# Frojdholm/rayrs

Measured on AMD Instinct MI355X. Metric: Mray/s (primary+secondary) on 1M-tri scene @1024spp, higher is better.
Workload: dtype f64

## Files before the change

### include/rayrs_hip.h

```cpp
#ifndef RAYRS_HIP_H
#define RAYRS_HIP_H

#include <stdint.h>

#ifdef __cplusplus
extern "C" {
#endif

typedef enum {
    RAYRS_OK = 0,
    RAYRS_INVALID_ARG = -1,
    RAYRS_HIP_ERROR = -2,
    RAYRS_OOM = -3,
    RAYRS_NO_DEVICE = -4,
    RAYRS_UNSUPPORTED = -5,
    RAYRS_IO_ERROR = -6,
    RAYRS_RCCL_ERROR = -7
} rayrs_status;

const char* rayrs_strerror(int status);
const char* rayrs_last_error(void);


enum {
// ... 3 lines not shown
    RAYRS_MAT_GLASS = 3,
    RAYRS_MAT_COOK_TORRANCE = 4,
    RAYRS_MAT_COOK_TORRANCE_REFRACT = 5,
    RAYRS_MAT_COOK_TORRANCE_GLASS = 6,
    RAYRS_MAT_PLASTIC = 7,
    RAYRS_MAT_NO_REFLECT = 8
};

typedef struct {
    int32_t kind;
    int32_t metallic;
    double color[3];
    double spec_color[3];
    double alpha;
    double ior;
    double r0[3];
} rayrs_material;

typedef struct {
    int32_t emissive;
    int32_t pad;
    double strength;
    double color[3];
} rayrs_emission;

enum { RAYRS_AXIS_X = 0, RAYRS_AXIS_XREV = 1, RAYRS_AXIS_Y = 2, RAYRS_AXIS_YREV = 3, RAYRS_AXIS_Z = 4, RAYRS_AXIS_ZREV = 5 };

enum { RAYRS_BVH_MIDPOINT = 0, RAYRS_BVH_SAH = 1 };


typedef struct rayrs_objects rayrs_objects;

int rayrs_objects_create(rayrs_objects** out);
void rayrs_objects_destroy(rayrs_objects* objs);
uint64_t rayrs_objects_len(const rayrs_objects* objs);

int rayrs_object_sphere(rayrs_objects* objs, double radius, const double origin[3], const rayrs_material* mat,
                        const rayrs_emission* emission);
int rayrs_object_plane(rayrs_objects* objs, int axis, double umin, double umax, double vmin, double vmax, double pos,
                       const rayrs_material* mat, const rayrs_emission* emission);
int rayrs_object_triangle(rayrs_objects* objs, const double p1[3], const double p2[3], const double p3[3],
                          const rayrs_material* mat, const rayrs_emission* emission);
int rayrs_object_from_triangles_f32(rayrs_objects* objs, const float* verts, uint32_t nverts, const uint32_t* idx,
                                    uint32_t ntris, const rayrs_material* mat, const rayrs_emission* emission);
int rayrs_object_from_triangles_f64(rayrs_objects* objs, const double* verts, uint32_t nverts, const uint32_t* idx,
                                    uint32_t ntris, const rayrs_material* mat, const rayrs_emission* emission);
int rayrs_object_from_spheres(rayrs_objects* objs, double radius, const double* centers, uint32_t n,
                              const rayrs_material* mat, const rayrs_emission* emission);
int rayrs_object_box_geom(rayrs_objects* objs, const double lower_left[3], const double upper_right[3],
                          const rayrs_material* mat, const rayrs_emission* emission);


typedef struct rayrs_scene rayrs_scene;

int rayrs_scene_new(const rayrs_objects* objs, double z_near, double z_far, int heuristic, uint32_t splits,
                    uint32_t hdri_w, uint32_t hdri_h, const float* hdri_rgb, int device, rayrs_scene** out);
void rayrs_scene_destroy(rayrs_scene* scene);

typedef struct {
    uint64_t n_objects;
    uint32_t n_interior;
    uint32_t n_prims;
    uint32_t root_ref;
    uint32_t depth;
    uint32_t compact;
    uint32_t n_surfaces;
    uint32_t node_bytes;
    uint32_t prim_bytes;
    uint64_t device_bytes;
    double root_box[6];
    double build_seconds;
    uint32_t n_wide;
    uint32_t wide_root_ref;
    uint32_t wide_depth;
    uint32_t local_pool;
    uint32_t gate_n_wide;
    uint32_t gate_root_ref;
    uint32_t gate_depth;
    uint32_t hot_n_wide;
    uint32_t hot_root_ref;
    uint32_t hot_depth;
    uint32_t hot_first;
    uint32_t hot_count;
    uint32_t hot_pad;
    double hot_box[6];
} rayrs_scene_info_t;

int rayrs_scene_info(const rayrs_scene* scene, rayrs_scene_info_t* info);
int rayrs_scene_clone_to_device(const rayrs_scene* scene, int device, rayrs_scene** out);
int rayrs_scene_device(const rayrs_scene* scene);
int rayrs_scene_export_bvh(const rayrs_scene* scene, double* child_box, uint32_t* child_ref, uint32_t* prim_object);
int rayrs_scene_export_wide(const rayrs_scene* scene, double* wide_box, uint32_t* wide_ref);
int rayrs_scene_export_gate_tree(const rayrs_scene* scene, double* wide_box, uint32_t* wide_ref);
int rayrs_scene_export_hot_tree(const rayrs_scene* scene, double* wide_box, uint32_t* wide_ref);


typedef struct {
    double origin[3];
    double e_x[3];
    double e_y[3];
    double z[3];
    double width, height;
    uint32_t ppc;
    uint32_t x_pixels;
    uint32_t y_pixels;
} rayrs_camera;

int rayrs_camera_new(const double origin[3], const double up[3], const double lookat[3], double fov, double width,
                     double height, uint32_t ppi, rayrs_camera* out);


enum { RAYRS_OUT_F32 = 0, RAYRS_OUT_F64 = 1 };

typedef struct {
    uint32_t spp;
    uint32_t max_bounces;
    uint64_t seed;
    uint32_t sample_chunk;
    uint32_t tile_rank, tile_ranks;
    uint32_t out_format;
    uint32_t count_work;
    uint32_t fast_traversal;
} rayrs_render_params;

typedef struct {
    uint64_t rays;
    uint64_t paths;
    uint64_t nan_pixels;
    uint64_t neg_pixels;
    uint64_t interior_visits;
    uint64_t tri_tests;
    uint64_t sphere_tests;
    uint64_t plane_tests;
    uint64_t escaped_paths;
    uint64_t step_wave, step_lane, inner_wave, leaf_wave;
    uint64_t interior_ticks, leaf_ticks;
    double kernel_ms;
    double total_ms;
    uint64_t kernel_launches;
    double trace_ms;
    uint64_t refill_ticks;
    uint64_t surface_hits[8];
    uint64_t direct_rays;
    double hit_ms, miss_ms;
    uint32_t local_pool;
    uint32_t exact_walk;
    uint32_t hot_group;
    uint32_t stats_pad;
    uint64_t pre_rays;
    uint64_t pre_root_records;
    uint64_t hot_lane;
    uint64_t hot_prim_tests;
    uint64_t hot_tri_divided;
} rayrs_render_stats;

uint32_t rayrs_frame_sample_chunk(uint32_t x_pixels, uint32_t y_pixels, uint32_t spp, uint32_t requested);

int rayrs_render(rayrs_scene* scene, const rayrs_camera* camera, const rayrs_render_params* params, void* out_host,
                 rayrs_render_stats* stats);

int rayrs_render_launch(rayrs_scene* scene, const rayrs_camera* camera, const rayrs_render_params* params,
                        void* out_device, void* hip_stream);
int rayrs_render_finish(rayrs_scene* scene, rayrs_render_stats* stats);

int rayrs_render_multi(rayrs_scene* const* scenes, uint32_t n, const rayrs_camera* camera,
                       const rayrs_render_params* params, void* out_host, rayrs_render_stats* stats);

typedef struct {
    uint32_t pool_slots;
    uint32_t local_pool;
} rayrs_tuning;
int rayrs_scene_set_tuning(rayrs_scene* scene, const rayrs_tuning* tuning);

typedef struct rayrs_film rayrs_film;

typedef struct {
    uint32_t sample_chunk;
    uint32_t max_bounces;
    uint64_t seed;
    uint32_t tile_rank, tile_ranks;
    uint32_t fast_traversal;
    uint32_t pad;
} rayrs_film_params;

typedef struct {
    uint64_t samples;
    uint64_t full_chunks;
    uint64_t rays, paths;
    uint64_t nan_pixels, neg_pixels;
    uint64_t unconverged, nonfinite;
    uint32_t closed;
    uint32_t pad;
} rayrs_film_status;

int rayrs_film_create(rayrs_scene* scene, const rayrs_camera* camera, const rayrs_film_params* params, rayrs_film** out);
void rayrs_film_destroy(rayrs_film* film);
int rayrs_film_render(rayrs_film* film, uint32_t n, rayrs_render_stats* pass_stats);
int rayrs_film_render_adaptive(rayrs_film* film, uint32_t n, double tau, uint32_t max_tile_samples,
                               uint64_t* active_tiles, rayrs_render_stats* pass_stats);
uint64_t rayrs_film_tile_samples(rayrs_film* film, uint32_t* out, uint64_t cap);
int rayrs_film_read(rayrs_film* film, uint32_t out_format, void* out_host);
int rayrs_film_status_get(rayrs_film* film, double tau, rayrs_film_status* out);
uint64_t rayrs_film_state_bytes(const rayrs_film* film);
int rayrs_film_state_get(rayrs_film* film, void* out_host, uint64_t cap);
int rayrs_film_state_set(rayrs_film* film, const void* in_host, uint64_t bytes);


int rayrs_render_features(rayrs_scene* scene, const rayrs_camera* camera, uint32_t samples, uint64_t seed, uint32_t tile_rank,
                          uint32_t tile_ranks, uint32_t fast_traversal, double* normal, double* albedo, double* depth,
                          double* coverage, uint32_t* object);
int rayrs_film_features(rayrs_film* film, uint32_t samples, double* normal, double* albedo, double* depth, double* coverage,
                        uint32_t* object);
int rayrs_film_denoise(rayrs_film* film, uint32_t feature_samples, uint32_t levels, double kn, double ka, double kz, double kc,
                       uint32_t out_format, void* out_host);
int rayrs_image_denoise(int device, uint32_t w, uint32_t h, const double* color, const double* normal, const double* albedo,
                        const double* depth, uint32_t levels, double kn, double ka, double kz, double kc, double* out);

#define RAYRS_ABI_VERSION 7
uint32_t rayrs_abi_version(void);

uint32_t rayrs_abi_layout(uint32_t* out, uint32_t cap);


const char* rayrs_io_last_error(void);
void rayrs_buffer_free(void* p);

int rayrs_ply_load(const char* path, float** verts, uint32_t* nverts, uint32_t** idx, uint32_t* ntris);
int rayrs_ply_save(const char* path, const float* verts, uint32_t nverts, const uint32_t* idx, uint32_t ntris,
                   int binary);
int rayrs_obj_load(const char* path, double** verts, uint32_t* nverts, uint32_t** idx, uint32_t* ntris);
int rayrs_obj_load_spheres(const char* path, double** centers, uint32_t* n);
// ... 11 lines not shown
```

### rayrs_amd/_ffi.py

```python
import ctypes as C
import os

_HERE = os.path.dirname(os.path.abspath(__file__))
LIB_PATH = os.environ.get("RAYRS_HIP_LIB") or os.path.join(_HERE, "librayrs_hip.so")

SYMBOLS = [
    "rayrs_strerror", "rayrs_last_error",
    "rayrs_objects_create", "rayrs_objects_destroy", "rayrs_objects_len",
    "rayrs_object_sphere", "rayrs_object_plane", "rayrs_object_triangle",
    "rayrs_object_from_triangles_f32", "rayrs_object_from_triangles_f64",
    "rayrs_object_from_spheres", "rayrs_object_box_geom",
    "rayrs_scene_new", "rayrs_scene_destroy", "rayrs_scene_info", "rayrs_scene_export_bvh",
    "rayrs_scene_export_wide", "rayrs_scene_export_gate_tree", "rayrs_scene_export_hot_tree", "rayrs_scene_clone_to_device", "rayrs_scene_device", "rayrs_scene_set_tuning",
    "rayrs_camera_new",
    "rayrs_frame_sample_chunk", "rayrs_render", "rayrs_render_launch", "rayrs_render_finish", "rayrs_render_multi",
    "rayrs_film_create", "rayrs_film_destroy", "rayrs_film_render", "rayrs_film_read", "rayrs_film_status_get",
    "rayrs_film_state_bytes", "rayrs_film_state_get", "rayrs_film_state_set",
    "rayrs_film_render_adaptive", "rayrs_film_tile_samples",
    "rayrs_render_features", "rayrs_film_features", "rayrs_film_denoise", "rayrs_image_denoise",
    "rayrs_abi_layout", "rayrs_abi_version",
    "rayrs_io_last_error", "rayrs_buffer_free", "rayrs_ply_load", "rayrs_ply_save", "rayrs_obj_load", "rayrs_obj_load_spheres",
    "rayrs_hdr_load", "rayrs_hdr_save", "rayrs_image_to_bytes", "rayrs_ppm_save", "rayrs_png_save",
]


PRIVATE_SYMBOLS = ["rayrs_test_math", "rayrs_test_rng", "rayrs_test_intersect", "rayrs_test_trace", "rayrs_test_path_trace", "rayrs_test_material", "rayrs_test_background",
                   "rayrs_lab_set", "rayrs_lab_round_ms", "rayrs_lab_multi_rehearse"]


class MaterialDesc(C.Structure):
    _fields_ = [("kind", C.c_int32), ("metallic", C.c_int32), ("color", C.c_double * 3),
                ("spec_color", C.c_double * 3), ("alpha", C.c_double), ("ior", C.c_double),
                ("r0", C.c_double * 3)]


class EmissionDesc(C.Structure):
    _fields_ = [("emissive", C.c_int32), ("pad", C.c_int32), ("strength", C.c_double),
                ("color", C.c_double * 3)]


class CameraDesc(C.Structure):
    _fields_ = [("origin", C.c_double * 3), ("e_x", C.c_double * 3), ("e_y", C.c_double * 3),
                ("z", C.c_double * 3), ("width", C.c_double), ("height", C.c_double),
                ("ppc", C.c_uint32), ("x_pixels", C.c_uint32), ("y_pixels", C.c_uint32)]


class SceneInfo(C.Structure):
    _fields_ = [("n_objects", C.c_uint64), ("n_interior", C.c_uint32), ("n_prims", C.c_uint32),
                ("root_ref", C.c_uint32), ("depth", C.c_uint32), ("compact", C.c_uint32),
                ("n_surfaces", C.c_uint32), ("node_bytes", C.c_uint32), ("prim_bytes", C.c_uint32),
                ("device_bytes", C.c_uint64), ("root_box", C.c_double * 6),
                ("build_seconds", C.c_double), ("n_wide", C.c_uint32), ("wide_root_ref", C.c_uint32),
                ("wide_depth", C.c_uint32), ("local_pool", C.c_uint32), ("gate_n_wide", C.c_uint32),
                ("gate_root_ref", C.c_uint32), ("gate_depth", C.c_uint32),
                ("hot_n_wide", C.c_uint32), ("hot_root_ref", C.c_uint32), ("hot_depth", C.c_uint32),
                ("hot_first", C.c_uint32), ("hot_count", C.c_uint32), ("hot_pad", C.c_uint32),
                ("hot_box", C.c_double * 6)]


class RenderParams(C.Structure):
    _fields_ = [("spp", C.c_uint32), ("max_bounces", C.c_uint32), ("seed", C.c_uint64),
                ("sample_chunk", C.c_uint32), ("tile_rank", C.c_uint32), ("tile_ranks", C.c_uint32),
                ("out_format", C.c_uint32), ("count_work", C.c_uint32), ("fast_traversal", C.c_uint32)]


class RenderStats(C.Structure):
    _fields_ = [("rays", C.c_uint64), ("paths", C.c_uint64), ("nan_pixels", C.c_uint64),
                ("neg_pixels", C.c_uint64), ("interior_visits", C.c_uint64), ("tri_tests", C.c_uint64),
                ("sphere_tests", C.c_uint64), ("plane_tests", C.c_uint64), ("escaped_paths", C.c_uint64),
                ("step_wave", C.c_uint64), ("step_lane", C.c_uint64), ("inner_wave", C.c_uint64),
                ("leaf_wave", C.c_uint64), ("interior_ticks", C.c_uint64), ("leaf_ticks", C.c_uint64),
                ("kernel_ms", C.c_double), ("total_ms", C.c_double), ("kernel_launches", C.c_uint64),
                ("trace_ms", C.c_double), ("refill_ticks", C.c_uint64),
                ("surface_hits", C.c_uint64 * 8), ("direct_rays", C.c_uint64), ("hit_ms", C.c_double), ("miss_ms", C.c_double),
                ("local_pool", C.c_uint32), ("exact_walk", C.c_uint32), ("hot_group", C.c_uint32),
                ("stats_pad", C.c_uint32), ("pre_rays", C.c_uint64), ("pre_root_records", C.c_uint64), ("hot_lane", C.c_uint64),
                ("hot_prim_tests", C.c_uint64), ("hot_tri_divided", C.c_uint64)]

    def as_dict(self):
        d = {n: getattr(self, n) for n, _ in self._fields_}
        d["surface_hits"] = list(self.surface_hits)
        return d


class Tuning(C.Structure):
    _fields_ = [("pool_slots", C.c_uint32), ("local_pool", C.c_uint32)]


class FilmParams(C.Structure):
    _fields_ = [("sample_chunk", C.c_uint32), ("max_bounces", C.c_uint32), ("seed", C.c_uint64),
                ("tile_rank", C.c_uint32), ("tile_ranks", C.c_uint32), ("fast_traversal", C.c_uint32), ("pad", C.c_uint32)]


class FilmStatus(C.Structure):
    _fields_ = [("samples", C.c_uint64), ("full_chunks", C.c_uint64), ("rays", C.c_uint64), ("paths", C.c_uint64),
                ("nan_pixels", C.c_uint64), ("neg_pixels", C.c_uint64), ("unconverged", C.c_uint64),
                ("nonfinite", C.c_uint64), ("closed", C.c_uint32), ("pad", C.c_uint32)]

    def as_dict(self):
        return {n: getattr(self, n) for n, _ in self._fields_ if n != "pad"}


class LabTuning(C.Structure):
    _fields_ = [("refill_min", C.c_uint32), ("leaf_min", C.c_uint32), ("static_pct", C.c_uint32),
                ("stack_lds", C.c_uint32), ("hot_records", C.c_uint32), ("trav_blocks_per_cu", C.c_uint32),
                ("eager_light", C.c_uint32), ("local_reserve", C.c_uint32), ("local_segment_items", C.c_uint32),
                ("force_rccl", C.c_uint32), ("gate_tree", C.c_uint32), ("hot_group", C.c_uint32), ("leaf_wait", C.c_uint32), ("flat_blocks_per_cu", C.c_uint32)]


ABI_VERSION = 7

ABI_STRUCTS = [MaterialDesc, EmissionDesc, CameraDesc, SceneInfo, RenderParams, RenderStats, Tuning, FilmParams, FilmStatus]

_lib = None


def lib():
    global _lib
    if _lib is not None:
        return _lib
    if not os.path.exists(LIB_PATH):
        raise RuntimeError(
            f"{LIB_PATH} is missing: build it with `python -c 'import __graft_entry__ as g; g.build()'` "
            "(make -C rayrs_amd/csrc). There is no CPU fallback.")
    L = C.CDLL(LIB_PATH)
    L.rayrs_abi_version.argtypes = []
    L.rayrs_abi_version.restype = C.c_uint32
    if L.rayrs_abi_version() != ABI_VERSION:
        raise RuntimeError(f"{LIB_PATH} has RAYRS_ABI_VERSION {L.rayrs_abi_version()}, this binding was written against "
                           f"{ABI_VERSION}: rebuild the library (make -C rayrs_amd/csrc)")
    dp = C.POINTER(C.c_double)
    vp = C.c_void_p
    L.rayrs_strerror.restype = C.c_char_p
    L.rayrs_strerror.argtypes = [C.c_int]
    L.rayrs_last_error.restype = C.c_char_p
    L.rayrs_objects_create.argtypes = [C.POINTER(vp)]
    L.rayrs_objects_destroy.argtypes = [vp]
    L.rayrs_objects_destroy.restype = None
    L.rayrs_objects_len.argtypes = [vp]
    L.rayrs_objects_len.restype = C.c_uint64
    mp, ep = C.POINTER(MaterialDesc), C.POINTER(EmissionDesc)
    L.rayrs_object_sphere.argtypes = [vp, C.c_double, dp, mp, ep]
    L.rayrs_object_plane.argtypes = [vp, C.c_int] + [C.c_double] * 5 + [mp, ep]
    L.rayrs_object_triangle.argtypes = [vp, dp, dp, dp, mp, ep]
    L.rayrs_object_from_triangles_f32.argtypes = [vp, vp, C.c_uint32, vp, C.c_uint32, mp, ep]
    L.rayrs_object_from_triangles_f64.argtypes = [vp, vp, C.c_uint32, vp, C.c_uint32, mp, ep]
    L.rayrs_object_from_spheres.argtypes = [vp, C.c_double, vp, C.c_uint32, mp, ep]
    L.rayrs_object_box_geom.argtypes = [vp, dp, dp, mp, ep]
    L.rayrs_scene_new.argtypes = [vp, C.c_double, C.c_double, C.c_int, C.c_uint32, C.c_uint32, C.c_uint32, vp,
                                  C.c_int, C.POINTER(vp)]
    L.rayrs_scene_destroy.argtypes = [vp]
    L.rayrs_scene_destroy.restype = None
    L.rayrs_scene_info.argtypes = [vp, C.POINTER(SceneInfo)]
    L.rayrs_scene_export_bvh.argtypes = [vp, vp, vp, vp]
    L.rayrs_scene_export_wide.argtypes = [vp, vp, vp]
    L.rayrs_scene_export_gate_tree.argtypes = [vp, vp, vp]
    L.rayrs_scene_export_hot_tree.argtypes = [vp, vp, vp]
    L.rayrs_scene_clone_to_device.argtypes = [vp, C.c_int, C.POINTER(vp)]
    L.rayrs_scene_device.argtypes = [vp]
# ... 82 lines not shown
```

### rayrs_amd/csrc/abi.cpp

```cpp
#include <hip/hip_runtime.h>

#include <cmath>
#include <cstddef>
#include <cstdlib>
#include <cstring>
#include <memory>
#include <new>
#include <stdexcept>
#include <string>
#include <vector>

#include "../../include/rayrs_hip.h"
#include "film.h"
#include "kernels.h"
#include "local_pool.h"
#include "rayrs_lab.h"
#include "scene_host.hpp"
#include "scene_internal.hpp"
#include "wavefront.h"

using namespace rayrs;

namespace {
thread_local std::string g_last_error;
// ... 217 lines not shown
    for (const SurfaceDev& sf : s->surfaces) ls.kind_mask |= 1u << (uint32_t)sf.kind;
    s->local_ok = true;
}

extern "C++" int rayrs::scene_upload(rayrs_scene* s) {
    HIP_TRY(hipSetDevice(s->device));
    hipDeviceProp_t prop;
    HIP_TRY(hipGetDeviceProperties(&prop, s->device));
    s->cu_count = prop.multiProcessorCount;
    const FlatScene& f = s->flat;
    for (int x = 0; x < 3; x++) {
        const WalkTree& t = s->tree(x);
        if (x == 2 && !f.has_hot) continue;
        HIP_TRY(s->trav[x].d_nodes.upload(t.node_bytes.data(), t.node_bytes.size()));
    }
    if (f.has_hot) HIP_TRY(s->d_hot.upload(&f.hot, sizeof(HotGroupDev)));
    HIP_TRY(s->d_prims.upload(f.prim_bytes.data(), f.prim_bytes.size()));
    HIP_TRY(s->d_surfaces.upload(s->surfaces.data(), s->surfaces.size() * sizeof(SurfaceDev)));
    HIP_TRY(s->d_hdri.upload(f.hdri_quads.data(), f.hdri_quads.size() * sizeof(float)));
    HIP_TRY(s->d_counters.reserve(sizeof(Counters)));
    for (auto& e : s->ev) HIP_TRY(e.create());
    s->device_bytes = f.walk.node_bytes.size() + f.gate.node_bytes.size() + (f.has_hot ? f.gate_hot.node_bytes.size() : 0) + f.prim_bytes.size() + s->surfaces.size() * sizeof(SurfaceDev) +
                      f.hdri_quads.size() * sizeof(float);
    RAYRS_TRY(scene_configure_traversal(s));
    HIP_TRY(s->pool.d_ctl.reserve(sizeof(WfCtl)));
    HIP_TRY(s->pool.h_live.alloc(2 * sizeof(uint32_t)));
    for (auto& e : s->pool.ev_batch) HIP_TRY(e.create());
    HIP_TRY(s->d_next_item.reserve(sizeof(unsigned long long)));
    if (s->local_ok) {
        HIP_TRY(lp_configure());
        HIP_TRY(lp_occupancy(s->flat.compact, s->local.n_prims, (uint32_t)s->surfaces.size(), &s->local_blocks_per_cu));
        if (s->local_blocks_per_cu < 1) s->local_blocks_per_cu = 1;
        if (s->local_blocks_per_cu > (int)LP_WPS) s->local_blocks_per_cu = (int)LP_WPS;
        HIP_TRY(s->d_local_items.reserve(LOCAL_MAX_SEGMENTS * sizeof(unsigned long long)));
    }
    return RAYRS_OK;
}

int rayrs_scene_new(const rayrs_objects* objs, double z_near, double z_far, int heuristic, uint32_t splits,
                    uint32_t hdri_w, uint32_t hdri_h, const float* hdri_rgb, int device, rayrs_scene** out) {
    RAYRS_GUARDED({
    if (!objs || !out) return RAYRS_INVALID_ARG;
    *out = nullptr;
    std::unique_ptr<rayrs_scene> s(new rayrs_scene());
    RAYRS_TRY(build_flat_scene(objs->list, z_near, z_far, heuristic, splits, hdri_w, hdri_h, hdri_rgb, &s->flat));
    if (std::max(s->flat.walk.depth, s->flat.gate.depth) > 4096u) {
        g_last_error = "walk tree needs " + std::to_string(std::max(s->flat.walk.depth, s->flat.gate.depth)) + " stack entries (limit 4096)";
        return RAYRS_UNSUPPORTED;
    }
    s->surfaces = objs->list.surfaces;
    s->n_objects = objs->list.objs.size();
    s->device = device;
    scene_configure_local(s.get());
    if (device >= 0) RAYRS_TRY(scene_upload(s.get()));
    *out = s.release();
    return RAYRS_OK;
    })
}

int rayrs_scene_info(const rayrs_scene* scene, rayrs_scene_info_t* info) {
    if (!scene || !info) return RAYRS_INVALID_ARG;
    const FlatScene& f = scene->flat;
    std::memset(info, 0, sizeof(*info));
    info->n_objects = scene->n_objects;
    info->n_interior = f.n_interior();
    info->n_prims = f.n_prims();
    info->root_ref = f.root_ref;
    info->depth = f.depth;
    info->compact = f.compact ? 1u : 0u;
    info->n_surfaces = (uint32_t)scene->surfaces.size();
    info->node_bytes = f.compact ? (uint32_t)sizeof(Node4F32) : (uint32_t)sizeof(Node4F64);
    info->n_wide = f.walk.n();
    info->wide_root_ref = f.walk.root_ref;
    info->wide_depth = f.walk.depth;
    info->gate_n_wide = f.gate.n();
    info->gate_root_ref = f.gate.root_ref;
    info->gate_depth = f.gate.depth;
    if (f.has_hot) {
        info->hot_n_wide = f.gate_hot.n();
        info->hot_root_ref = f.gate_hot.root_ref;
        info->hot_depth = f.gate_hot.depth;
        info->hot_first = f.hot.first;
        info->hot_count = f.hot.count;
        for (int i = 0; i < 6; i++) info->hot_box[i] = f.hot.box[i];
    }
    info->local_pool = (scene->local_ok && scene->tuning.local_pool != 1u) ? 1u : 0u;
    info->prim_bytes = 4u * (f.compact ? PRIM_DWORDS_COMPACT : PRIM_DWORDS_FULL);
    info->device_bytes = scene->device_bytes;
    for (int i = 0; i < 6; i++) info->root_box[i] = f.root_box[i];
    info->build_seconds = f.build_seconds;
    return RAYRS_OK;
}

int rayrs_scene_export_bvh(const rayrs_scene* scene, double* child_box, uint32_t* child_ref, uint32_t* prim_object) {
    if (!scene) return RAYRS_INVALID_ARG;
    const FlatScene& f = scene->flat;
    if (child_box && !f.child_box.empty()) std::memcpy(child_box, f.child_box.data(), f.child_box.size() * 8);
    if (child_ref && !f.child_ref.empty()) std::memcpy(child_ref, f.child_ref.data(), f.child_ref.size() * 4);
    if (prim_object && !f.prim_object.empty())
        std::memcpy(prim_object, f.prim_object.data(), f.prim_object.size() * 4);
    return RAYRS_OK;
}

static int export_tree(const WalkTree& t, double* wide_box, uint32_t* wide_ref) {
    if (wide_box && !t.box.empty()) std::memcpy(wide_box, t.box.data(), t.box.size() * 8);
    if (wide_ref && !t.ref.empty()) std::memcpy(wide_ref, t.ref.data(), t.ref.size() * 4);
    return RAYRS_OK;
}

int rayrs_scene_export_wide(const rayrs_scene* scene, double* wide_box, uint32_t* wide_ref) {
    return scene ? export_tree(scene->flat.walk, wide_box, wide_ref) : RAYRS_INVALID_ARG;
}

int rayrs_scene_export_gate_tree(const rayrs_scene* scene, double* wide_box, uint32_t* wide_ref) {
    return scene ? export_tree(scene->flat.gate, wide_box, wide_ref) : RAYRS_INVALID_ARG;
}

int rayrs_scene_export_hot_tree(const rayrs_scene* scene, double* wide_box, uint32_t* wide_ref) {
    return scene && scene->flat.has_hot ? export_tree(scene->flat.gate_hot, wide_box, wide_ref) : RAYRS_INVALID_ARG;
}

int rayrs_scene_clone_to_device(const rayrs_scene* scene, int device, rayrs_scene** out) {
    RAYRS_GUARDED({
        if (!scene || !out || device < 0) return RAYRS_INVALID_ARG;
        *out = nullptr;
        std::unique_ptr<rayrs_scene> s(new rayrs_scene());
        s->flat = scene->flat;
        s->surfaces = scene->surfaces;
        s->n_objects = scene->n_objects;
        s->tuning = scene->tuning;
        s->lab = scene->lab;
        s->device = device;
        scene_configure_local(s.get());
        RAYRS_TRY(scene_upload(s.get()));
        *out = s.release();
        return RAYRS_OK;
    })
}

int rayrs_scene_device(const rayrs_scene* scene) { return scene ? scene->device : -1; }

static int scene_quiesce(rayrs_scene* scene) {
    if (scene->device >= 0) {
        HIP_TRY(hipSetDevice(scene->device));
        if (scene->pending && scene->last_stream) {
            HIP_TRY(hipStreamSynchronize(scene->last_stream));
            scene->pending = false;
        }
    }
    return RAYRS_OK;
}

rayrs_scene::~rayrs_scene() {
    if (device < 0) return;
    (void)hipSetDevice(device);
    if (pending && last_stream) (void)hipStreamSynchronize(last_stream);
}

int rayrs_scene_set_tuning(rayrs_scene* scene, const rayrs_tuning* tuning) {
    if (!scene || !tuning) return RAYRS_INVALID_ARG;
    if (tuning->local_pool > 1u) return RAYRS_INVALID_ARG;
    RAYRS_TRY(scene_quiesce(scene));
    scene->tuning = *tuning;
    return RAYRS_OK;
}

// ... 8 lines not shown
}
#endif

static int round_event(rayrs_scene::Pool& pl, uint32_t r, uint32_t k, hipStream_t stream) {
    while (pl.ev_round.size() < 4 * (size_t)(r + 1)) {
        Event e;
        HIP_TRY(e.create());
        pl.ev_round.push_back(std::move(e));
    }
    HIP_TRY(hipEventRecord(pl.ev_round[4 * (size_t)r + k], stream));
    return RAYRS_OK;
}

static int round_ms(const rayrs_scene* scene, uint32_t r, float ms[3]) {
    const Event* e = &scene->pool.ev_round[4 * (size_t)r];
    ms[1] = ms[2] = 0.f;
    HIP_TRY(hipEventElapsedTime(&ms[0], e[0], e[1]));
    if (scene->last_local) return RAYRS_OK;
    HIP_TRY(hipEventElapsedTime(&ms[1], e[1], e[2]));
    HIP_TRY(hipEventElapsedTime(&ms[2], e[2], e[3]));
    return RAYRS_OK;
}

extern "C" int rayrs_lab_round_ms(rayrs_scene* scene, float* out, uint32_t cap_rounds) {
    if (!scene || scene->device < 0 || scene->pending) return RAYRS_INVALID_ARG;
    HIP_TRY(hipSetDevice(scene->device));
    for (uint32_t r = 0; r < scene->pool.timed_rounds && r < cap_rounds && out; r++) RAYRS_TRY(round_ms(scene, r, out + 3 * r));
    return (int)scene->pool.timed_rounds;
}

int rayrs_lab_set(rayrs_scene* scene, const rayrs_lab_tuning* lab) {
    if (!scene || !lab) return RAYRS_INVALID_ARG;
    if (lab->stack_lds > 64u) return RAYRS_INVALID_ARG;
    if (lab->hot_group != 0u && lab->hot_group != 0xffffffffu) return RAYRS_INVALID_ARG;
    if (lab->static_pct > 100u || lab->refill_min > 64u || lab->leaf_min > 64u || lab->leaf_wait > 64u || lab->flat_blocks_per_cu > 64u || lab->eager_light > 1u || lab->force_rccl > 1u || lab->gate_tree > 1u)
        return RAYRS_INVALID_ARG;
    if (lab->local_reserve != 0u && (lab->local_reserve < 8u || lab->local_reserve > 4096u)) return RAYRS_INVALID_ARG;
    if (lab->local_segment_items != 0u && lab->local_segment_items < 65536u) return RAYRS_INVALID_ARG;
    RAYRS_TRY(scene_quiesce(scene));
    scene->lab = *lab;
    if (scene->device >= 0) return scene_configure_traversal(scene);
    return RAYRS_OK;
}

uint32_t rayrs_frame_sample_chunk(uint32_t x_pixels, uint32_t y_pixels, uint32_t spp, uint32_t requested) {
    if (spp == 0) return 0;
    uint64_t chunk = requested ? requested : 4u;
    const uint64_t pixels = (uint64_t)((x_pixels + 7u) / 8u) * ((y_pixels + 7u) / 8u) * 64u;
    while (chunk < spp && pixels * ((spp + chunk - 1) / chunk) > (1ull << 30)) chunk *= 2;
    return chunk >= spp ? 0u : (uint32_t)chunk;
}

uint32_t rayrs_abi_version(void) { return RAYRS_ABI_VERSION; }

uint32_t rayrs_abi_layout(uint32_t* out, uint32_t cap) {
    std::vector<uint32_t> t;
    t.push_back(RAYRS_ABI_VERSION);
#define RAYRS_STRUCT(T, N) t.push_back((uint32_t)sizeof(T)), t.push_back(N)
#define RAYRS_FIELD(T, F) t.push_back((uint32_t)offsetof(T, F))
    RAYRS_STRUCT(rayrs_material, 7);
    RAYRS_FIELD(rayrs_material, kind), RAYRS_FIELD(rayrs_material, metallic), RAYRS_FIELD(rayrs_material, color);
    RAYRS_FIELD(rayrs_material, spec_color), RAYRS_FIELD(rayrs_material, alpha), RAYRS_FIELD(rayrs_material, ior);
    RAYRS_FIELD(rayrs_material, r0);
    RAYRS_STRUCT(rayrs_emission, 4);
    RAYRS_FIELD(rayrs_emission, emissive), RAYRS_FIELD(rayrs_emission, pad), RAYRS_FIELD(rayrs_emission, strength);
    RAYRS_FIELD(rayrs_emission, color);
    RAYRS_STRUCT(rayrs_camera, 9);
    RAYRS_FIELD(rayrs_camera, origin), RAYRS_FIELD(rayrs_camera, e_x), RAYRS_FIELD(rayrs_camera, e_y);
    RAYRS_FIELD(rayrs_camera, z), RAYRS_FIELD(rayrs_camera, width), RAYRS_FIELD(rayrs_camera, height);
    RAYRS_FIELD(rayrs_camera, ppc), RAYRS_FIELD(rayrs_camera, x_pixels), RAYRS_FIELD(rayrs_camera, y_pixels);
    RAYRS_STRUCT(rayrs_scene_info_t, 26);
    RAYRS_FIELD(rayrs_scene_info_t, n_objects), RAYRS_FIELD(rayrs_scene_info_t, n_interior);
    RAYRS_FIELD(rayrs_scene_info_t, n_prims), RAYRS_FIELD(rayrs_scene_info_t, root_ref);
    RAYRS_FIELD(rayrs_scene_info_t, depth), RAYRS_FIELD(rayrs_scene_info_t, compact);
    RAYRS_FIELD(rayrs_scene_info_t, n_surfaces), RAYRS_FIELD(rayrs_scene_info_t, node_bytes);
    RAYRS_FIELD(rayrs_scene_info_t, prim_bytes), RAYRS_FIELD(rayrs_scene_info_t, device_bytes);
    RAYRS_FIELD(rayrs_scene_info_t, root_box), RAYRS_FIELD(rayrs_scene_info_t, build_seconds);
    RAYRS_FIELD(rayrs_scene_info_t, n_wide), RAYRS_FIELD(rayrs_scene_info_t, wide_root_ref);
    RAYRS_FIELD(rayrs_scene_info_t, wide_depth), RAYRS_FIELD(rayrs_scene_info_t, local_pool);
    RAYRS_FIELD(rayrs_scene_info_t, gate_n_wide), RAYRS_FIELD(rayrs_scene_info_t, gate_root_ref);
    RAYRS_FIELD(rayrs_scene_info_t, gate_depth);
    RAYRS_FIELD(rayrs_scene_info_t, hot_n_wide), RAYRS_FIELD(rayrs_scene_info_t, hot_root_ref);
    RAYRS_FIELD(rayrs_scene_info_t, hot_depth), RAYRS_FIELD(rayrs_scene_info_t, hot_first);
    RAYRS_FIELD(rayrs_scene_info_t, hot_count), RAYRS_FIELD(rayrs_scene_info_t, hot_pad);
    RAYRS_FIELD(rayrs_scene_info_t, hot_box);
    RAYRS_STRUCT(rayrs_render_params, 9);
    RAYRS_FIELD(rayrs_render_params, spp), RAYRS_FIELD(rayrs_render_params, max_bounces);
    RAYRS_FIELD(rayrs_render_params, seed), RAYRS_FIELD(rayrs_render_params, sample_chunk);
    RAYRS_FIELD(rayrs_render_params, tile_rank), RAYRS_FIELD(rayrs_render_params, tile_ranks);
    RAYRS_FIELD(rayrs_render_params, out_format), RAYRS_FIELD(rayrs_render_params, count_work);
    RAYRS_FIELD(rayrs_render_params, fast_traversal);
    RAYRS_STRUCT(rayrs_render_stats, 33);
    RAYRS_FIELD(rayrs_render_stats, rays), RAYRS_FIELD(rayrs_render_stats, paths);
    RAYRS_FIELD(rayrs_render_stats, nan_pixels), RAYRS_FIELD(rayrs_render_stats, neg_pixels);
    RAYRS_FIELD(rayrs_render_stats, interior_visits), RAYRS_FIELD(rayrs_render_stats, tri_tests);
    RAYRS_FIELD(rayrs_render_stats, sphere_tests), RAYRS_FIELD(rayrs_render_stats, plane_tests);
    RAYRS_FIELD(rayrs_render_stats, escaped_paths), RAYRS_FIELD(rayrs_render_stats, step_wave);
    RAYRS_FIELD(rayrs_render_stats, step_lane), RAYRS_FIELD(rayrs_render_stats, inner_wave);
    RAYRS_FIELD(rayrs_render_stats, leaf_wave), RAYRS_FIELD(rayrs_render_stats, interior_ticks);
    RAYRS_FIELD(rayrs_render_stats, leaf_ticks), RAYRS_FIELD(rayrs_render_stats, kernel_ms);
    RAYRS_FIELD(rayrs_render_stats, total_ms), RAYRS_FIELD(rayrs_render_stats, kernel_launches);
    RAYRS_FIELD(rayrs_render_stats, trace_ms), RAYRS_FIELD(rayrs_render_stats, refill_ticks);
    RAYRS_FIELD(rayrs_render_stats, surface_hits), RAYRS_FIELD(rayrs_render_stats, direct_rays);
    RAYRS_FIELD(rayrs_render_stats, hit_ms), RAYRS_FIELD(rayrs_render_stats, miss_ms);
    RAYRS_FIELD(rayrs_render_stats, local_pool), RAYRS_FIELD(rayrs_render_stats, exact_walk);
    RAYRS_FIELD(rayrs_render_stats, hot_group), RAYRS_FIELD(rayrs_render_stats, stats_pad);
    RAYRS_FIELD(rayrs_render_stats, pre_rays), RAYRS_FIELD(rayrs_render_stats, pre_root_records);
    RAYRS_FIELD(rayrs_render_stats, hot_lane);
    RAYRS_FIELD(rayrs_render_stats, hot_prim_tests), RAYRS_FIELD(rayrs_render_stats, hot_tri_divided);
    RAYRS_STRUCT(rayrs_tuning, 2);
    RAYRS_FIELD(rayrs_tuning, pool_slots), RAYRS_FIELD(rayrs_tuning, local_pool);
    RAYRS_STRUCT(rayrs_film_params, 7);
    RAYRS_FIELD(rayrs_film_params, sample_chunk), RAYRS_FIELD(rayrs_film_params, max_bounces);
    RAYRS_FIELD(rayrs_film_params, seed), RAYRS_FIELD(rayrs_film_params, tile_rank);
    RAYRS_FIELD(rayrs_film_params, tile_ranks), RAYRS_FIELD(rayrs_film_params, fast_traversal);
    RAYRS_FIELD(rayrs_film_params, pad);
    RAYRS_STRUCT(rayrs_film_status, 10);
    RAYRS_FIELD(rayrs_film_status, samples), RAYRS_FIELD(rayrs_film_status, full_chunks);
    RAYRS_FIELD(rayrs_film_status, rays), RAYRS_FIELD(rayrs_film_status, paths);
    RAYRS_FIELD(rayrs_film_status, nan_pixels), RAYRS_FIELD(rayrs_film_status, neg_pixels);
    RAYRS_FIELD(rayrs_film_status, unconverged), RAYRS_FIELD(rayrs_film_status, nonfinite);
    RAYRS_FIELD(rayrs_film_status, closed), RAYRS_FIELD(rayrs_film_status, pad);
#undef RAYRS_STRUCT
#undef RAYRS_FIELD
    for (uint32_t i = 0; i < cap && i < t.size(); i++) out[i] = t[i];
    return (uint32_t)t.size();
}


int rayrs_camera_new(const double origin[3], const double up[3], const double lookat[3], double fov, double width,
                     double height, uint32_t ppi, rayrs_camera* out) {
    return camera_new(origin, up, lookat, fov, width, height, ppi, out);
}


extern "C++" SceneDev rayrs::make_scene_dev(const rayrs_scene* s, bool exact) {
    SceneDev sc;
    std::memset(&sc, 0, sizeof(sc));
    const int which = s->walk_index(exact);
    const WalkTree& t = s->tree(which);
    const rayrs_scene::Walk& w = s->trav[which];
    sc.hot = which == 2 ? s->d_hot.as<HotGroupDev>() : nullptr;
    sc.nodes = w.d_nodes.as<>();
    sc.prims = s->d_prims.as<>();
    sc.surfaces = s->d_surfaces.as<SurfaceDev>();
    sc.hdri = s->d_hdri.as<float>();
    sc.hdri_w = s->flat.hdri_w;
    sc.hdri_h = s->flat.hdri_h;
    sc.hdri_wm1 = (double)(s->flat.hdri_w - 1u);
    sc.hdri_hm1 = (double)(s->flat.hdri_h - 1u);
    sc.root_ref = t.root_ref;
    sc.stack_depth = t.depth ? t.depth : 1;
    sc.stack_lds = w.stack_lds;
    sc.hot_records = w.hot_records;
    sc.leafq = w.leafq;
    sc.n_surfaces = (uint32_t)s->surfaces.size();
    for (int i = 0; i < 6; i++) sc.root_box[i] = s->flat.root_box[i];
    sc.t0 = s->flat.t0;
    sc.t1 = s->flat.t1;
    sc.exact = exact ? 1u : 0u;
    return sc;
}

constexpr double RAYRS_FAR_DIAGONALS = 8.0;
constexpr double RAYRS_FAR_PRIMITIVES = 4096.0;
extern "C++" bool rayrs::camera_is_far(const rayrs_scene* s, const rayrs_camera* c) {
    const double* b = s->flat.root_box;
    double d2 = 0.0, e2 = 0.0;
    for (int a = 0; a < 3; a++) {
        const double lo = b[2 * a], hi = b[2 * a + 1], o = c->origin[a];
        const double out = o < lo ? lo - o : (o > hi ? o - hi : 0.0);
        d2 += out * out;
        e2 += (hi - lo) * (hi - lo);
    }
    const double small = s->flat.small_extent;
    return d2 > RAYRS_FAR_DIAGONALS * RAYRS_FAR_DIAGONALS * e2 || (small > 0.0 && d2 > RAYRS_FAR_PRIMITIVES * RAYRS_FAR_PRIMITIVES * small * small);
}

extern "C++" CameraDev rayrs::make_camera_dev(const rayrs_camera* c) {
    CameraDev cam;
    std::memset(&cam, 0, sizeof(cam));
    for (int i = 0; i < 3; i++) {
        cam.origin[i] = c->origin[i];
        cam.e_x[i] = c->e_x[i];
        cam.e_y[i] = c->e_y[i];
        cam.z[i] = c->z[i];
    }
    cam.width = c->width;
    cam.height = c->height;
    cam.ppc = (double)c->ppc;
    cam.W = c->x_pixels;
    cam.H = c->y_pixels;
    return cam;
}

extern "C++" uint32_t rayrs::trav_settings(const rayrs_scene* s, bool exact, uint32_t np, RenderDev& rp) {
    const rayrs_lab_tuning& lab = s->lab;
    rp.refill_min = lab.refill_min ? lab.refill_min : 52u;
    rp.leaf_min = lab.leaf_min ? lab.leaf_min : (exact ? 48u : lab.gate_tree ? 32u : 24u);
    rp.leaf_wait = lab.leaf_wait ? lab.leaf_wait : 16u;
    uint32_t trav_bpc = (uint32_t)s->trav[s->walk_index(exact)].blocks_per_cu;
    if (lab.trav_blocks_per_cu && lab.trav_blocks_per_cu < trav_bpc) trav_bpc = lab.trav_blocks_per_cu;
    const uint32_t blocks = (uint32_t)s->cu_count * trav_bpc;
    const uint32_t static_pct = lab.static_pct ? lab.static_pct : 50u;
    const uint64_t n_waves = (uint64_t)blocks * 4u;
    rp.static_windows = (uint32_t)((uint64_t)(np / wf_window_slots()) * static_pct / 100u / n_waves * n_waves);
    return blocks;
}

extern "C++" WfDev rayrs::pool_wf(const DevBuf& block, uint32_t np, const DevBuf& ctl, uint32_t trav_blocks, const DevBuf& spill) {
    WfDev wf;
    std::memset(&wf, 0, sizeof(wf));
    wf.slots = block.as<PathSlot>();
    wf.light = reinterpret_cast<double*>(wf.slots + np);
    wf.state = reinterpret_cast<uint8_t*>(wf.light + (size_t)np * 4u);
    wf.ctl = ctl.as<WfCtl>();
    wf.np = np;
    wf.trav_threads = trav_blocks * 256u;
    wf.stack_spill = spill.as<uint32_t>();
    return wf;
}

struct FramePlan {
    SceneDev sc;
    CameraDev cam;
    RenderDev rp;
    bool exact, eager_light, use_local;
    uint64_t partial_need;
    uint64_t tile_items, seg_tiles, seg_items;
    uint32_t local_blocks;
    uint64_t live_total;
    uint32_t np, trav_blocks, flat_blocks;
    size_t spill_words;
    bool is_film;
    FilmPassDev film;
};

static RenderDev make_render_dev(const rayrs_scene* scene, const rayrs_camera* camera, const rayrs_render_params* params, uint32_t sample0,
                                 const FilmPassDev* film, void* out_device) {
    RenderDev rp;
    std::memset(&rp, 0, sizeof(rp));
    rp.spp = params->spp;
    rp.sample0 = sample0;
// ... 90 lines not shown
        lp.item_count = rp.total_items - lp.item_base < p.seg_items ? rp.total_items - lp.item_base : p.seg_items;
        RenderDev rseg = rp;
        rseg.partial_item0 = lp.item_base;
        const uint64_t share = lp.item_count / ((uint64_t)p.local_blocks * 4u * 16u);
        lp.reserve = (uint32_t)(share < 8u ? 8u : share > 256u ? 256u : share);
        if (scene->lab.local_reserve) lp.reserve = scene->lab.local_reserve;
        lp.pad = 0;
        RAYRS_TRY(round_event(pl, (uint32_t)seg, 0, stream));
        HIP_TRY(lp_launch(scene->flat.compact, rp.count_work != 0u, p.sc, scene->local, p.cam, rseg, lp, p.local_blocks, stream));
        RAYRS_TRY(round_event(pl, (uint32_t)seg, 1, stream));
        const uint32_t seg_lt0 = (uint32_t)(seg * p.seg_tiles), seg_n_lt = (uint32_t)(lp.item_count / p.tile_items);
        HIP_TRY(p.is_film ? launch_film_accumulate(p.cam, rseg, p.film, seg_lt0, seg_n_lt, stream) : launch_resolve(p.cam, rseg, seg_lt0, seg_n_lt, stream));
        pl.timed_rounds = (uint32_t)seg + 1;
    }
    scene->rounds = (uint32_t)n_seg;
    return RAYRS_OK;
}

static int enqueue_streaming(rayrs_scene* scene, const FramePlan& p, const WfDev& wf, hipStream_t stream) {
    rayrs_scene::Pool& pl = scene->pool;
    const RenderDev& rp = p.rp;
    uint32_t* h_live = pl.h_live.as<uint32_t>();
    HIP_TRY(wf_launch_init(wf, (uint32_t)p.live_total, stream));
    HIP_TRY(wf_launch_gen(scene->flat.compact, p.sc, p.cam, rp, wf, p.flat_blocks, stream));
    h_live[0] = h_live[1] = (uint32_t)p.live_total;
    constexpr uint32_t MAX_TIMED = 8192;
    uint32_t it = 0;
    uint32_t batch = 16;
    for (uint32_t b = 0;; b++) {
        for (uint32_t k = 0; k < batch; k++, it++) {
            const bool timed = it < MAX_TIMED;
            if (timed) RAYRS_TRY(round_event(pl, it, 0, stream));
            HIP_TRY(wf_launch_trav(scene->flat.compact, rp.count_work != 0u, p.sc, rp, wf, p.trav_blocks, stream));
            if (timed) RAYRS_TRY(round_event(pl, it, 1, stream));
            HIP_TRY(wf_launch_hit(scene->flat.compact, p.eager_light, p.sc, p.cam, rp, wf, p.flat_blocks, stream));
            if (timed) RAYRS_TRY(round_event(pl, it, 2, stream));
            HIP_TRY(wf_launch_miss(scene->flat.compact, p.eager_light, p.sc, p.cam, rp, wf, p.flat_blocks, stream));
            if (timed) {
                RAYRS_TRY(round_event(pl, it, 3, stream));
                pl.timed_rounds = it + 1;
            }
        }
        HIP_TRY(hipMemcpyAsync(&h_live[b & 1u], &wf.ctl->live_slots, sizeof(uint32_t), hipMemcpyDeviceToHost, stream));
        HIP_TRY(hipEventRecord(pl.ev_batch[b & 1u], stream));
        if (b > 0) {
            HIP_TRY(hipEventSynchronize(pl.ev_batch[(b - 1u) & 1u]));
            const uint64_t seen = h_live[(b - 1u) & 1u];
            if (seen == 0u) break;
            batch = seen * 8u < p.live_total ? 4u : 16u;
        }
        if (it > (1u << 26)) {
            g_last_error = "path rounds did not terminate";
            return RAYRS_HIP_ERROR;
        }
    }
    scene->rounds = it;
    return RAYRS_OK;
}

extern "C++" int rayrs::render_enqueue(rayrs_scene* scene, const rayrs_camera* camera, const rayrs_render_params* params, uint32_t sample0,
                                       const FilmPassDev* film, void* out_device, void* hip_stream) {
    RAYRS_GUARDED({
    if (!scene || !camera || !params || (!out_device && !film)) return RAYRS_INVALID_ARG;
    if (scene->device < 0) return RAYRS_NO_DEVICE;
    if (params->spp == 0 || camera->x_pixels == 0 || camera->y_pixels == 0) return RAYRS_INVALID_ARG;
    if (camera->x_pixels > 65535u || camera->y_pixels > 65535u) return RAYRS_UNSUPPORTED;
    if (params->max_bounces > 8000u) return RAYRS_UNSUPPORTED;
    if (params->spp > SLOT_SAMPLE_MASK || sample0 > SLOT_SAMPLE_MASK - params->spp) return RAYRS_UNSUPPORTED;
    if (params->tile_ranks == 0 || params->tile_rank >= params->tile_ranks) return RAYRS_INVALID_ARG;
    if (params->out_format != RAYRS_OUT_F32 && params->out_format != RAYRS_OUT_F64) return RAYRS_INVALID_ARG;
    if (params->fast_traversal > 1u) return RAYRS_INVALID_ARG;
    HIP_TRY(hipSetDevice(scene->device));
    hipStream_t stream = reinterpret_cast<hipStream_t>(hip_stream);
    if (scene->pending) {
        HIP_TRY(hipStreamSynchronize(scene->last_stream));
        scene->pending = false;
    }

    FramePlan p;
    RAYRS_TRY(plan_frame(scene, camera, params, sample0, film, out_device, p));
    p.is_film = film != nullptr;
    p.film = film ? *film : FilmPassDev{};
    scene->last_exact = p.exact;

    rayrs_scene::Pool& pl = scene->pool;
    HIP_TRY(scene->d_partial.reserve((size_t)p.partial_need * 3 * sizeof(double)));
    p.rp.partial = scene->d_partial.as<double>();
    HIP_TRY(scene->d_local_light.reserve((size_t)p.local_blocks * 4u * LP_PATHS_PER_WAVE * 4 * sizeof(double)));
    HIP_TRY(pl.block.reserve((size_t)p.np * POOL_SLOT_BYTES));
    HIP_TRY(pl.d_wave_items.reserve((size_t)p.flat_blocks * 4u * 2 * sizeof(unsigned long long)));
    HIP_TRY(pl.d_stack_spill.reserve(p.spill_words * sizeof(uint32_t)));
    WfDev wf = pool_wf(pl.block, p.np, pl.d_ctl, p.trav_blocks, pl.d_stack_spill);
    wf.n_flat_waves = p.flat_blocks * 4u;
    wf.wave_items = pl.d_wave_items.as<unsigned long long>();

    pl.timed_rounds = 0;
    HIP_TRY(hipMemsetAsync(p.rp.counters, 0, sizeof(Counters), stream));
    HIP_TRY(hipMemsetAsync(p.rp.next_item, 0, sizeof(unsigned long long), stream));
    if (p.use_local) HIP_TRY(hipMemsetAsync(scene->d_local_items.as<>(), 0, LOCAL_MAX_SEGMENTS * sizeof(unsigned long long), stream));
    HIP_TRY(hipEventRecord(scene->ev[0], stream));
    scene->rounds = 0;
    scene->last_local = p.use_local;
    if (p.rp.total_items > 0) RAYRS_TRY(p.use_local ? enqueue_local(scene, p, stream) : enqueue_streaming(scene, p, wf, stream));
    HIP_TRY(hipEventRecord(scene->ev[1], stream));
    if (!p.use_local) HIP_TRY(p.is_film ? launch_film_accumulate(p.cam, p.rp, p.film, 0u, p.rp.n_local_tiles, stream) : launch_resolve(p.cam, p.rp, 0u, p.rp.n_local_tiles, stream));
    HIP_TRY(hipEventRecord(scene->ev[2], stream));
    scene->last_stream = stream;
    scene->pending = true;
    return RAYRS_OK;
    })
}

int rayrs_render_launch(rayrs_scene* scene, const rayrs_camera* camera, const rayrs_render_params* params,
                        void* out_device, void* hip_stream) {
    if (!out_device) return RAYRS_INVALID_ARG;
    return render_enqueue(scene, camera, params, 0u, nullptr, out_device, hip_stream);
}

int rayrs_render_finish(rayrs_scene* scene, rayrs_render_stats* stats) {
    if (!scene) return RAYRS_INVALID_ARG;
    if (scene->device < 0) return RAYRS_NO_DEVICE;
    if (!scene->pending) return RAYRS_INVALID_ARG;
    HIP_TRY(hipSetDevice(scene->device));
    HIP_TRY(hipEventSynchronize(scene->ev[2]));
    scene->pending = false;
    if (stats) {
        Counters c;
        HIP_TRY(scene->d_counters.download(&c, sizeof(c)));
        std::memset(stats, 0, sizeof(*stats));
        stats->rays = c.rays;
        stats->paths = c.paths;
        stats->nan_pixels = c.nan_pixels;
        stats->neg_pixels = c.neg_pixels;
        stats->interior_visits = c.interior_visits;
        stats->tri_tests = c.tri_tests;
        stats->sphere_tests = c.sphere_tests;
        stats->plane_tests = c.plane_tests;
        stats->escaped_paths = c.escaped_paths;
        stats->step_wave = c.step_wave, stats->step_lane = c.step_lane, stats->inner_wave = c.inner_wave;
        stats->leaf_wave = c.leaf_wave, stats->interior_ticks = c.interior_ticks, stats->leaf_ticks = c.leaf_ticks;
        stats->refill_ticks = c.refill_ticks;
        for (int k = 0; k < 8; k++) stats->surface_hits[k] = c.surface_hits[k];
        stats->direct_rays = c.direct_rays;
        stats->pre_rays = c.pre_rays, stats->pre_root_records = c.pre_root_records, stats->hot_lane = c.hot_lane;
        stats->hot_prim_tests = c.hot_prim_tests, stats->hot_tri_divided = c.hot_tri_divided;
        float ms = 0.f;
        HIP_TRY(hipEventElapsedTime(&ms, scene->ev[0], scene->ev[1]));
        stats->trace_ms = ms;
        HIP_TRY(hipEventElapsedTime(&ms, scene->ev[0], scene->ev[2]));
        stats->total_ms = ms;
        const uint32_t timed_rounds = scene->pool.timed_rounds;
        double t = 0.0, h = 0.0, m = 0.0;
        for (uint32_t r = 0; r < timed_rounds; r++) {
            float k[3];
            RAYRS_TRY(round_ms(scene, r, k));
            t += k[0], h += k[1], m += k[2];
        }
        if (timed_rounds && scene->rounds > timed_rounds) {
            const double f = (double)scene->rounds / (double)timed_rounds;
            t *= f, h *= f, m *= f;
        }
        stats->kernel_ms = t;
        stats->hit_ms = h, stats->miss_ms = m;
        stats->local_pool = scene->last_local ? 1u : 0u;
        stats->exact_walk = (scene->last_exact || scene->last_local) ? 1u : 0u;
        stats->hot_group = (!scene->last_local && scene->last_exact && scene->walk_index(true) == 2) ? 1u : 0u;
        stats->kernel_launches = (uint64_t)scene->rounds;
    }
    return RAYRS_OK;
}

int rayrs_render(rayrs_scene* scene, const rayrs_camera* camera, const rayrs_render_params* params, void* out_host,
                 rayrs_render_stats* stats) {
    if (!scene || !camera || !params || !out_host) return RAYRS_INVALID_ARG;
    if (scene->device < 0) return RAYRS_NO_DEVICE;
    HIP_TRY(hipSetDevice(scene->device));
    const size_t elem = params->out_format == RAYRS_OUT_F64 ? 8 : 4;
    const size_t bytes = (size_t)camera->x_pixels * camera->y_pixels * 3 * elem;
    DevBuf d_out;
    HIP_TRY(d_out.upload(out_host, bytes));
    RAYRS_TRY(rayrs_render_launch(scene, camera, params, d_out.as<>(), nullptr));
    RAYRS_TRY(rayrs_render_finish(scene, stats));
    HIP_TRY(d_out.download(out_host, bytes));
    return RAYRS_OK;
}

}
```

### rayrs_amd/csrc/device_path.h

```cpp
#pragma once
#include <hip/hip_runtime.h>

#include "../../include/rayrs_hip.h"
#include "../../include/rayrs_numeric.h"
#include "layout.h"

namespace rayrs {

#define RR_DEV __device__ __forceinline__

struct V3 {
    double x, y, z;
};

RR_DEV uint32_t lanes_below(unsigned long long mask) {
    return __builtin_amdgcn_mbcnt_hi((uint32_t)(mask >> 32), __builtin_amdgcn_mbcnt_lo((uint32_t)mask, 0u));
}

RR_DEV V3 mk(double x, double y, double z) { return V3{x, y, z}; }
RR_DEV V3 v_add(V3 a, V3 b) { return mk(a.x + b.x, a.y + b.y, a.z + b.z); }
RR_DEV V3 v_sub(V3 a, V3 b) { return mk(a.x - b.x, a.y - b.y, a.z - b.z); }
RR_DEV V3 v_mul(V3 a, V3 b) { return mk(a.x * b.x, a.y * b.y, a.z * b.z); }
RR_DEV V3 v_scale(V3 a, double s) { return mk(a.x * s, a.y * s, a.z * s); }
RR_DEV V3 v_div(V3 a, double s) {
// ... 451 lines not shown
        else x = gsrc[0], y = gsrc[1], z = gsrc[2], r = gsrc[12];
        r0 = r.x, r1 = r.y, r2 = r.z, r3 = r.w;
        h0 = slab_f64(x, y, z, nx, ny, nz, o, inv, tmin, tmax, e0);
        if (in_lds) x = lsrc[3], y = lsrc[4], z = lsrc[5];
        else x = gsrc[3], y = gsrc[4], z = gsrc[5];
        h1 = slab_f64(x, y, z, nx, ny, nz, o, inv, tmin, tmax, e1);
        if (in_lds) x = lsrc[6], y = lsrc[7], z = lsrc[8];
        else x = gsrc[6], y = gsrc[7], z = gsrc[8];
        h2 = slab_f64(x, y, z, nx, ny, nz, o, inv, tmin, tmax, e2);
        if (in_lds) x = lsrc[9], y = lsrc[10], z = lsrc[11];
        else x = gsrc[9], y = gsrc[10], z = gsrc[11];
        h3 = slab_f64(x, y, z, nx, ny, nz, o, inv, tmin, tmax, e3);
    }
    asm volatile("" : "+v"(r0), "+v"(r1), "+v"(r2), "+v"(r3));
    const unsigned long long m0 = __builtin_amdgcn_ballot_w64(h0), m1 = __builtin_amdgcn_ballot_w64(h1);
    const unsigned long long m2 = __builtin_amdgcn_ballot_w64(h2), m3 = __builtin_amdgcn_ballot_w64(h3);
    const unsigned long long q0 = __builtin_amdgcn_ballot_w64(r0 >= REF_LEAF_BASE), q1 = __builtin_amdgcn_ballot_w64(r1 >= REF_LEAF_BASE);
    const unsigned long long q2 = __builtin_amdgcn_ballot_w64(r2 >= REF_LEAF_BASE), q3 = __builtin_amdgcn_ballot_w64(r3 >= REF_LEAF_BASE);
#define RR_LANE_BIT(mask) __builtin_amdgcn_inverse_ballot_w64(mask)
    const bool i0 = RR_LANE_BIT(m0 & ~q0), i1 = RR_LANE_BIT(m1 & ~q1), i2 = RR_LANE_BIT(m2 & ~q2), i3 = RR_LANE_BIT(m3 & ~q3);
    const bool l0 = RR_LANE_BIT(m0 & q0), l1 = RR_LANE_BIT(m1 & q1), l2 = RR_LANE_BIT(m2 & q2), l3 = RR_LANE_BIT(m3 & q3);
#undef RR_LANE_BIT
    const int ki1 = (int)i0, ki2 = ki1 + (int)i1, ki3 = ki2 + (int)i2, n_int = ki3 + (int)i3;
    const int kl1 = (int)l0, kl2 = kl1 + (int)l1, kl3 = kl2 + (int)l2, n_leaf = kl3 + (int)l3;
    const int sp = (int)((uint32_t)tv.sp & 0xffffu);
    const int lq = (int)((uint32_t)tv.sp >> 16);
    const int top = sp + n_int - 1;
    const int spare = (int)stack.cap;
    const int qbase = spare + 1 + lq;
    const int d0 = i0 ? top : (l0 ? qbase : spare);
    const int d1 = i1 ? top - ki1 : (l1 ? qbase + kl1 : spare);
    const int d2 = i2 ? top - ki2 : (l2 ? qbase + kl2 : spare);
    const int d3 = i3 ? top - ki3 : (l3 ? qbase + kl3 : spare);
    if (__ballot(n_int > 0 && (uint32_t)top > stack.cap) == 0ull) {
        stack.lds[d0 * 64] = r0;
        stack.lds[d1 * 64] = r1;
        stack.lds[d2 * 64] = r2;
        stack.lds[d3 * 64] = r3;
    } else {
        if (l0) stack.lds[d0 * 64] = r0;
        if (l1) stack.lds[d1 * 64] = r1;
        else if (i1 && ki1 > 0) stack.put(top - ki1, r1);
        if (l2) stack.lds[d2 * 64] = r2;
        else if (i2 && ki2 > 0) stack.put(top - ki2, r2);
        if (l3) stack.lds[d3 * 64] = r3;
        else if (i3 && ki3 > 0) stack.put(top - ki3, r3);
    }
    if (n_int > 0) {
        tv.cur = i0 ? r0 : i1 ? r1 : i2 ? r2 : r3;
        tv.sp = (int)(((uint32_t)(lq + n_leaf) << 16) | (uint32_t)top);
    } else if (sp > 0) {
        tv.cur = stack.get(sp - 1);
        tv.sp = (int)(((uint32_t)(lq + n_leaf) << 16) | (uint32_t)(sp - 1));
    } else {
        tv.cur = TRAV_DONE;
        tv.sp = (int)((uint32_t)(lq + n_leaf) << 16);
    }
}

template <bool COMPACT, bool COUNT>
RR_DEV void trav_leaf_step_defer(const SceneDev& sc, V3 o, V3 d, const LaneStack& stack, Trav& tv, WorkCount& wc) {
    const double tmin = sc.t0, tmax = sc.t1;
    tv.sp -= (int)LEAFQ_ONE;
    const uint32_t ref = defer_queue(stack)[((uint32_t)tv.sp >> 16) * 64u];
    const uint32_t first = (ref & 0x3fffffffu) >> 2;
    const uint32_t count = (ref & 3u) + 1u;
    if (COUNT) wc.leaf_prims = count;
    for (uint32_t k = 0; k < count; k++) {
        const uint32_t p = first + k;
        const PrimRec<COMPACT> r = load_prim<COMPACT>(sc.prims, p);
        if (COUNT) {
            const uint32_t kind = r.tag() & 3u;
            if (kind == PRIM_TRIANGLE) wc.tri++;
            else if (kind == PRIM_SPHERE) wc.sphere++;
            else wc.plane++;
        }
        double t;
        if (prim_intersect<COMPACT>(r, o, d, t) && t > tmin && t < tmax) {
            if (t < tv.best_t || (t == tv.best_t && p < tv.best_prim)) {
                tv.best_t = t;
                tv.best_prim = p;
            }
        }
    }
}


typedef const __attribute__((address_space(4))) HotGroupDev* HotPtr;
RR_DEV HotPtr hot_ptr(const SceneDev& sc) { return (HotPtr)sc.hot; }

RR_DEV bool hot_triangle_intersect(V3 p1, V3 e1, V3 e2, V3 o, V3 d, bool live, double& t, HotTally& ht) {
    const V3 tt = v_sub(o, p1);
    const V3 p = v_cross(d, e2);
    const V3 q = v_cross(tt, e1);
    const double den = v_dot(p, e1);
    const double n0 = v_dot(q, e2), n1 = v_dot(p, tt), n2 = v_dot(q, d);
    {
        const uint32_t dh = (uint32_t)(rr_f64_bits(den) >> 32);
        const unsigned long long opp0 = __builtin_amdgcn_ballot_w64((int)((uint32_t)(rr_f64_bits(n0) >> 32) ^ dh) < 0);
        const unsigned long long opp1 = __builtin_amdgcn_ballot_w64((int)((uint32_t)(rr_f64_bits(n1) >> 32) ^ dh) < 0);
        const unsigned long long opp2 = __builtin_amdgcn_ballot_w64((int)((uint32_t)(rr_f64_bits(n2) >> 32) ^ dh) < 0);
        const double aden = rr_fabs(den), a0 = rr_fabs(n0), a1 = rr_fabs(n1), a2 = rr_fabs(n2);
        const unsigned long long den_le = __builtin_amdgcn_ballot_w64(aden <= 0x1p500);
        const unsigned long long den_ge = __builtin_amdgcn_ballot_w64(aden >= 0x1p-500);
        const unsigned long long big0 = __builtin_amdgcn_ballot_w64(a0 >= 0x1p-500);
        const unsigned long long big1 = __builtin_amdgcn_ballot_w64(a1 >= 0x1p-500);
        const unsigned long long big2 = __builtin_amdgcn_ballot_w64(a2 >= 0x1p-500);
        const unsigned long long fin1 = __builtin_amdgcn_ballot_w64(a1 <= 0x1p500);
        const unsigned long long fin2 = __builtin_amdgcn_ballot_w64(a2 <= 0x1p500);
        const double two_den = aden * 2.0;
        const unsigned long long two1 = __builtin_amdgcn_ballot_w64(a1 >= two_den);
        const unsigned long long two2 = __builtin_amdgcn_ballot_w64(a2 >= two_den);
        const unsigned long long settled = (den_le & ((opp0 & big0) | (opp1 & big1) | (opp2 & big2))) |
                                           (den_le & den_ge & ((~opp1 & two1 & fin2) | (~opp2 & two2 & fin1)));
        if ((__builtin_amdgcn_ballot_w64(live) & ~settled) == 0ull) return false;
    }
    ht.divided += (uint32_t)__popcll(__builtin_amdgcn_ballot_w64(live));
    double dd, u, v;
    div3_by(n0, n1, n2, den, dd, u, v);
    const unsigned long long out = __builtin_amdgcn_ballot_w64(dd < 0.0) | __builtin_amdgcn_ballot_w64(u < 0.0) |
                                   __builtin_amdgcn_ballot_w64(v < 0.0) | __builtin_amdgcn_ballot_w64(u + v > 1.0);
    if (__builtin_amdgcn_inverse_ballot_w64(out)) return false;
    t = dd;
    return true;
}

RR_DEV bool uniform_box_entered(double x0, double x1, double y0, double y1, double z0, double z1, V3 o, V3 inv, double tmin,
                                double tmax) {
    const bool nx = inv.x < 0.0, ny = inv.y < 0.0, nz = inv.z < 0.0;
    const double ax = (x0 - o.x) * inv.x, bx = (x1 - o.x) * inv.x;
    const double ay = (y0 - o.y) * inv.y, by = (y1 - o.y) * inv.y;
    const double az = (z0 - o.z) * inv.z, bz = (z1 - o.z) * inv.z;
    double lo = tmin, hi = tmax;
    lo = rr_max(lo, nx ? bx : ax), hi = rr_min(hi, nx ? ax : bx);
    lo = rr_max(lo, ny ? by : ay), hi = rr_min(hi, ny ? ay : by);
    lo = rr_max(lo, nz ? bz : az), hi = rr_min(hi, nz ? az : bz);
    return !(hi <= lo);
}

template <bool COUNT>
RR_DEV void hot_group_step(const SceneDev& sc, V3 o, V3 d, bool owe, Trav& tv, WorkCount& wc, HotTally& ht) {
    const HotPtr h = hot_ptr(sc);
    const double tmin = sc.t0, tmax = sc.t1;
    const V3 inv = tv.inv;
    const bool entered = owe && uniform_box_entered(h->box[0], h->box[1], h->box[2], h->box[3], h->box[4], h->box[5], o, inv, tmin, tmax);
    const unsigned long long entered_mask = __builtin_amdgcn_ballot_w64(entered);
    ht.owed += (uint32_t)__popcll(__builtin_amdgcn_ballot_w64(owe));
    ht.entered += (uint32_t)__popcll(entered_mask);
    if (entered_mask == 0ull) return;
    const uint32_t first = h->first, count = h->count;
#pragma nounroll
    for (uint32_t k = 0; k < count; k++) {
        const uint32_t tag = h->prim[k].tag;
        const uint32_t kind = tag & 3u;
        double t = 0.0;
        bool hit;
        if (kind == PRIM_TRIANGLE) {
            if (COUNT && entered) wc.tri++;
            hit = hot_triangle_intersect(mk(h->prim[k].v[0], h->prim[k].v[1], h->prim[k].v[2]),
                                         mk(h->prim[k].v[3], h->prim[k].v[4], h->prim[k].v[5]),
                                         mk(h->prim[k].v[6], h->prim[k].v[7], h->prim[k].v[8]), o, d, entered, t, ht);
        } else if (kind == PRIM_SPHERE) {
            if (COUNT && entered) wc.sphere++;
            hit = sphere_intersect(h->prim[k].v[0], mk(h->prim[k].v[1], h->prim[k].v[2], h->prim[k].v[3]), o, d, t);
        } else {
            if (COUNT && entered) wc.plane++;
// ... 417 lines not shown
```

### rayrs_amd/csrc/layout.h

```cpp
#pragma once
#include <stdint.h>

namespace rayrs {

constexpr uint32_t REF_INTERIOR = 0u;
constexpr uint32_t REF_RANGE = 1u;
constexpr uint32_t REF_SINGLE = 2u;
constexpr uint32_t REF_NONE = 3u;

constexpr uint32_t PRIM_SPHERE = 0u;
constexpr uint32_t PRIM_PLANE = 1u;
constexpr uint32_t PRIM_TRIANGLE = 2u;

struct NodeF32 {
    float box[2][6];
    uint32_t ref[2];
    uint32_t pad[2];
};
struct NodeF64 {
    double box[2][6];
    uint32_t ref[2];
    uint32_t pad[6];
};
static_assert(sizeof(NodeF32) == 64, "NodeF32");
static_assert(sizeof(NodeF64) == 128, "NodeF64");

struct Node4F32 {
    float box[4][6];
    uint32_t ref[4];
    uint32_t pad[4];
};
struct Node4F64 {
    double box[4][6];
    uint32_t ref[4];
    uint32_t pad[12];
};
constexpr uint32_t WIDE_FRONT = 256;
constexpr uint32_t TRAV_LEAFQ = 8;
static_assert(sizeof(Node4F32) == 128, "Node4F32");
static_assert(sizeof(Node4F64) == 256, "Node4F64");

constexpr uint32_t PRIM_DWORDS_COMPACT = 12;
constexpr uint32_t PRIM_DWORDS_FULL = 20;

struct SurfaceDev {
    int32_t kind;
    int32_t metallic;
    double color[3];
    double ior;
    double ct_alpha2;
    double ct_ior;
    double ct_r0[3];
    double ct_color[3];
    double emit[3];
    int32_t emissive;
    int32_t pad;
};

struct HotPrim {
    double v[9];
    uint32_t tag;
    uint32_t pad;
};
struct HotGroupDev {
    double box[6];
    uint32_t first;
    uint32_t count;
    uint32_t pad[2];
    HotPrim prim[4];
    double root_box[4][6];
    uint32_t root_ref[4];
    uint32_t n_tri, n_sphere, n_plane, pad1;
};
static_assert(sizeof(HotPrim) == 80 && sizeof(HotGroupDev) == 384 + 192 + 32, "HotGroupDev");

struct SceneDev {
    const void* nodes;
    const void* prims;
    const SurfaceDev* surfaces;
    const float* hdri;
    uint32_t hdri_w, hdri_h;
    uint32_t root_ref;
    uint32_t stack_depth;
    uint32_t stack_lds;
    uint32_t hot_records;
    uint32_t n_surfaces;
    uint32_t leafq;
    double root_box[6];
    double t0, t1;
    double hdri_wm1, hdri_hm1;
    uint32_t exact, pad1;
    const HotGroupDev* hot;
};

struct CameraDev {
    double origin[3], e_x[3], e_y[3], z[3];
    double width, height, ppc;
    uint32_t W, H;
};

struct Counters {
    unsigned long long rays, paths, nan_pixels, neg_pixels;
    unsigned long long interior_visits, tri_tests, sphere_tests, plane_tests, escaped_paths;
    unsigned long long step_wave, step_lane, inner_wave, leaf_wave;
    unsigned long long interior_ticks, leaf_ticks, refill_ticks;
    unsigned long long surface_hits[8];
    unsigned long long direct_rays;
    unsigned long long pre_rays;
    unsigned long long pre_root_records;
    unsigned long long hot_lane;
    unsigned long long hot_prim_tests;
    unsigned long long hot_tri_divided;
#ifdef RAYRS_LAB_TICKS
    unsigned long long lab_ticks[16];
#endif
};

struct alignas(8) TileRef {
    uint32_t tile, samples;
};
static_assert(sizeof(TileRef) == 8, "TileRef");

struct RenderDev {
    uint32_t spp, max_bounces;
    uint64_t seed;
    uint32_t chunk, nchunks;
    uint32_t tile_rank, tile_ranks;
    uint32_t tiles_x, tiles_y;
    uint32_t n_local_tiles;
    uint32_t out_format;
    uint64_t total_items;
    double inv_nchunks, inv_tiles_x;
    uint32_t refill_min, leaf_min;
    uint32_t leaf_wait;
    uint32_t sample0;
    uint32_t static_windows;
    uint32_t count_work;
    double* partial;
    uint64_t partial_item0;
    unsigned long long* next_item;
    Counters* counters;
    void* out;
    const TileRef* tile_list;
};

#if defined(__HIPCC__)
#define RR_LAYOUT_FN __host__ __device__ static inline
#else
#define RR_LAYOUT_FN static inline
#endif
RR_LAYOUT_FN uint32_t udiv_by(uint32_t n, uint32_t d, double inv_d, uint32_t& rem) {
    uint32_t q = (uint32_t)((double)n * inv_d);
    int32_t r = (int32_t)(n - q * d);
    if (r < 0) q--, r += (int32_t)d;
    else if ((uint32_t)r >= d) q++, r -= (int32_t)d;
    rem = (uint32_t)r;
    return q;
}

RR_LAYOUT_FN void item_geometry(const RenderDev& rp, uint32_t item, uint32_t& row, uint32_t& col, uint32_t& s_begin,
                                uint32_t& s_end) {
    const uint32_t pit = item & 63u;
    uint32_t chunk, tile_col;
    const uint32_t lt = udiv_by(item >> 6, rp.nchunks, rp.inv_nchunks, chunk);
    uint32_t tile = lt * rp.tile_ranks + rp.tile_rank, s0 = rp.sample0;
    if (rp.tile_list) {
        const TileRef t = rp.tile_list[lt < rp.n_local_tiles ? lt : 0u];
        tile = t.tile, s0 = t.samples;
    }
    row = udiv_by(tile, rp.tiles_x, rp.inv_tiles_x, tile_col) * 8u + (pit >> 3);
    col = tile_col * 8u + (pit & 7u);
    const uint32_t w_end = s0 + rp.spp;
    s_begin = s0 + chunk * rp.chunk;
    s_end = s_begin + rp.chunk < w_end ? s_begin + rp.chunk : w_end;
// ... 4 lines not shown
```

### rayrs_amd/csrc/scene_host.cpp

```cpp
#include "scene_host.hpp"

#include <algorithm>
#include <chrono>
#include <cmath>
#include <cstddef>
#include <cstdlib>
#include <cstring>
#include <limits>

#include "../../include/rayrs_numeric.h"

namespace rayrs {


static bool in01(const double* c) {
    return c[0] >= 0.0 && c[0] <= 1.0 && c[1] >= 0.0 && c[1] <= 1.0 && c[2] >= 0.0 && c[2] <= 1.0;
}

int ObjectList::add_surface(const rayrs_material* m, const rayrs_emission* e) {
    if (!m) return RAYRS_INVALID_ARG;
    SurfaceDev s;
    std::memset(&s, 0, sizeof(s));
    s.kind = m->kind;
    if (m->kind < 0 || m->kind > RAYRS_MAT_NO_REFLECT) return RAYRS_INVALID_ARG;
// ... 643 lines not shown
    f.root_box[0] = root.xmin, f.root_box[1] = root.xmax, f.root_box[2] = root.ymin;
    f.root_box[3] = root.ymax, f.root_box[4] = root.zmin, f.root_box[5] = root.zmax;

    {
        std::vector<Aabb> prim_box(n);
        for (size_t p = 0; p < n; p++) prim_box[p] = b.boxes[f.prim_object[p]];
        build_walk_trees(f, prim_box);
        std::vector<double> ext(n);
        for (size_t p = 0; p < n; p++) {
            const Aabb& pb = prim_box[p];
            const double e = std::max(pb.xmax - pb.xmin, std::max(pb.ymax - pb.ymin, pb.zmax - pb.zmin));
            ext[p] = e > 0.0 ? e : std::numeric_limits<double>::infinity();
        }
        std::nth_element(ext.begin(), ext.begin() + (std::ptrdiff_t)(n / 20), ext.end());
        f.small_extent = std::isfinite(ext[n / 20]) ? ext[n / 20] : 0.0;
    }

    bool compact = boxes_f32_exact(f.gate) && boxes_f32_exact(f.walk) && boxes_f32_exact(f.gate_hot);
    for (size_t i = 0; i < n && compact; i++) {
        const Shape& s = objs.objs[i].geom;
        if (s.kind != PRIM_TRIANGLE) continue;
        const double v[9] = {s.p1.x, s.p1.y, s.p1.z, s.p2.x, s.p2.y, s.p2.z, s.p3.x, s.p3.y, s.p3.z};
        for (double c : v)
            if (!f32_exact(c)) {
                compact = false;
                break;
            }
    }
    f.compact = compact;
    for (WalkTree* t : {&f.gate, &f.walk, &f.gate_hot}) {
        if (compact) fill_nodes<Node4F32, float>(*t);
        else fill_nodes<Node4F64, double>(*t);
    }

    const uint32_t dw = compact ? PRIM_DWORDS_COMPACT : PRIM_DWORDS_FULL;
    f.prim_bytes.assign((size_t)n * dw * 4, 0);
    uint32_t* prims = reinterpret_cast<uint32_t*>(f.prim_bytes.data());
    for (size_t p = 0; p < n; p++) {
        const Object& o = objs.objs[f.prim_object[p]];
        const Shape& s = o.geom;
        uint32_t* rec = prims + p * dw;
        if (s.kind == PRIM_SPHERE) {
            put_f64(rec + 0, s.radius2);
            put_f64(rec + 2, s.origin.x);
            put_f64(rec + 4, s.origin.y);
            put_f64(rec + 6, s.origin.z);
        } else if (s.kind == PRIM_PLANE) {
            put_f64(rec + 0, s.u0);
            put_f64(rec + 2, s.u1);
            put_f64(rec + 4, s.v0);
            put_f64(rec + 6, s.v1);
            put_f64(rec + 8, s.pos);
        } else {
            const double v[9] = {s.p1.x, s.p1.y, s.p1.z, s.p2.x, s.p2.y, s.p2.z, s.p3.x, s.p3.y, s.p3.z};
            for (int k = 0; k < 9; k++) {
                if (compact)
                    put_f32(rec + k, (float)v[k]);
                else
                    put_f64(rec + 2 * k, v[k]);
            }
        }
        rec[dw - 1] = s.kind | (s.axis << 2) | (o.surface << 8);
    }

    if (f.has_hot) {
        for (uint32_t k = 0; k < f.hot.count; k++) {
            const Object& o = objs.objs[f.prim_object[f.hot.first + k]];
            const Shape& s = o.geom;
            HotPrim& hp = f.hot.prim[k];
            if (s.kind == PRIM_SPHERE) {
                hp.v[0] = s.radius2, hp.v[1] = s.origin.x, hp.v[2] = s.origin.y, hp.v[3] = s.origin.z;
            } else if (s.kind == PRIM_PLANE) {
                hp.v[0] = s.u0, hp.v[1] = s.u1, hp.v[2] = s.v0, hp.v[3] = s.v1, hp.v[4] = s.pos;
            } else {
                hp.v[0] = s.p1.x, hp.v[1] = s.p1.y, hp.v[2] = s.p1.z;
                hp.v[3] = s.p2.x - s.p1.x, hp.v[4] = s.p2.y - s.p1.y, hp.v[5] = s.p2.z - s.p1.z;
                hp.v[6] = s.p3.x - s.p1.x, hp.v[7] = s.p3.y - s.p1.y, hp.v[8] = s.p3.z - s.p1.z;
            }
            hp.tag = s.kind | (s.axis << 2) | (o.surface << 8);
            if (s.kind == PRIM_SPHERE) f.hot.n_sphere++;
            else if (s.kind == PRIM_PLANE) f.hot.n_plane++;
            else f.hot.n_tri++;
        }
        const WalkTree& t = f.gate_hot;
        const uint32_t r = t.root_ref & 0x3fffffffu;
        const double inf = std::numeric_limits<double>::infinity();
        for (int ch = 0; ch < 4; ch++) {
            const uint32_t ref = t.ref[(size_t)r * 4 + ch];
            f.hot.root_ref[ch] = ref;
            for (int k = 0; k < 6; k++)
                f.hot.root_box[ch][k] = (ref >> 30) == REF_NONE ? ((k & 1) ? -inf : inf) : t.box[((size_t)r * 4 + ch) * 6 + k];
        }
    }

    f.hdri_w = hdri_w;
    f.hdri_h = hdri_h;
    {
        std::vector<float> rgb((size_t)hdri_w * hdri_h * 3);
        for (size_t t = 0; t < rgb.size(); t++) {
            const double v = rr_max(rr_min((double)hdri_rgb[t], 3.0), 0.0);
            rgb[t] = (float)v;
        }
        f.hdri_quads.assign((size_t)hdri_w * hdri_h * 16, 0.f);
        for (uint32_t i = 0; i < hdri_h; i++) {
            const uint32_t i1 = i + 1 < hdri_h ? i + 1 : hdri_h - 1;
            for (uint32_t j = 0; j < hdri_w; j++) {
                const uint32_t j1 = j + 1 < hdri_w ? j + 1 : hdri_w - 1;
                const size_t src[4] = {(size_t)i * hdri_w + j, (size_t)i1 * hdri_w + j, (size_t)i * hdri_w + j1,
                                       (size_t)i1 * hdri_w + j1};
                float* q = &f.hdri_quads[((size_t)i * hdri_w + j) * 16];
                for (int k = 0; k < 4; k++)
                    for (int c = 0; c < 3; c++) q[k * 4 + c] = rgb[src[k] * 3 + c];
            }
        }
    }

    f.build_seconds = std::chrono::duration<double>(std::chrono::steady_clock::now() - t_begin).count();
    return RAYRS_OK;
}


static inline Vec3 sub(Vec3 a, Vec3 b) { return {a.x - b.x, a.y - b.y, a.z - b.z}; }
static inline Vec3 cross(Vec3 a, Vec3 b) {
    return {a.y * b.z - a.z * b.y, a.z * b.x - a.x * b.z, a.x * b.y - a.y * b.x};
}
static inline Vec3 unit(Vec3 a) {
    const double inv = 1.0 / rr_sqrt(a.x * a.x + a.y * a.y + a.z * a.z);
    return {a.x * inv, a.y * inv, a.z * inv};
}

int camera_new(const double origin[3], const double up[3], const double lookat[3], double fov, double width,
               double height, uint32_t ppi, rayrs_camera* out) {
    if (!origin || !up || !lookat || !out) return RAYRS_INVALID_ARG;
    if (!(fov > 0. && fov < 180.)) return RAYRS_INVALID_ARG;
    if (!(width > 0.) || !(height > 0.)) return RAYRS_INVALID_ARG;
    const Vec3 o{origin[0], origin[1], origin[2]}, u{up[0], up[1], up[2]}, la{lookat[0], lookat[1], lookat[2]};
    if (o.x == la.x && o.y == la.y && o.z == la.z) return RAYRS_INVALID_ARG;
    const uint32_t ppc = (uint32_t)std::round((double)ppi * 2.54);
    const Vec3 z = unit(sub(la, o));
    const Vec3 x = unit(cross(u, z));
    const Vec3 y = unit(cross(z, x));
    const double rad = fov * (RR_PI / 180.0);
    const double focal = width / rr_tan(rad / 2.);
    out->origin[0] = o.x, out->origin[1] = o.y, out->origin[2] = o.z;
    out->e_x[0] = x.x, out->e_x[1] = x.y, out->e_x[2] = x.z;
    out->e_y[0] = y.x, out->e_y[1] = y.y, out->e_y[2] = y.z;
    out->z[0] = focal * z.x, out->z[1] = focal * z.y, out->z[2] = focal * z.z;
    out->width = width;
    out->height = height;
    out->ppc = ppc;
    out->x_pixels = (uint32_t)std::round(width * (double)ppc);
    out->y_pixels = (uint32_t)std::round(height * (double)ppc);
    return RAYRS_OK;
}

}
```

### rayrs_amd/csrc/scene_host.hpp

```cpp
#pragma once
#include <cstdint>
#include <string>
#include <vector>

#include "../../include/rayrs_hip.h"
#include "layout.h"

namespace rayrs {

struct Vec3 {
    double x, y, z;
};

struct Aabb {
    double xmin, xmax, ymin, ymax, zmin, zmax;
};

struct Shape {
    uint32_t kind;
    uint32_t axis;
    double radius2;
    Vec3 origin;
    double u0, u1, v0, v1, pos;
    Vec3 p1, p2, p3;
};

struct Object {
    Shape geom;
    uint32_t surface;
};

struct ObjectList {
    std::vector<Object> objs;
    std::vector<SurfaceDev> surfaces;

    int add_surface(const rayrs_material* m, const rayrs_emission* e);
};

Aabb shape_bbox(const Shape& s);

struct WalkTree {
    std::vector<double> box;
    std::vector<uint32_t> ref;
    uint32_t root_ref = 0;
    uint32_t depth = 0;
    std::vector<uint8_t> node_bytes;
    uint32_t n() const { return (uint32_t)(ref.size() / 4); }
};

struct FlatScene {
    std::vector<double> child_box;
    std::vector<uint32_t> child_ref;
    std::vector<uint32_t> prim_object;
    uint32_t root_ref = 0;
    uint32_t depth = 0;
    WalkTree walk, gate, gate_hot;
    bool has_hot = false;
    HotGroupDev hot = {};
    double root_box[6] = {0, 0, 0, 0, 0, 0};
    bool compact = false;
    std::vector<uint8_t> prim_bytes;
    std::vector<float> hdri_quads;
    uint32_t hdri_w = 0, hdri_h = 0;
    double t0 = 0, t1 = 0;
    double build_seconds = 0;
    double small_extent = 0;
    uint32_t n_interior() const { return (uint32_t)(child_ref.size() / 2); }
    uint32_t n_prims() const { return (uint32_t)prim_object.size(); }
};

int build_flat_scene(const ObjectList& objs, double z_near, double z_far, int heuristic, uint32_t splits,
                     uint32_t hdri_w, uint32_t hdri_h, const float* hdri_rgb, FlatScene* out);

int camera_new(const double origin[3], const double up[3], const double lookat[3], double fov, double width,
               double height, uint32_t ppi, rayrs_camera* out);

}
```

### rayrs_amd/csrc/scene_internal.hpp

```cpp
#pragma once
#include <hip/hip_runtime.h>

#include <cstdint>
#include <string>
#include <vector>

#include "../../include/rayrs_hip.h"
#include "device_mem.hpp"
#include "film.h"
#include "local_pool.h"
#include "rayrs_lab.h"
#include "scene_host.hpp"
#include "wavefront.h"

struct rayrs_objects {
    rayrs::ObjectList list;
};

struct rayrs_scene {
    rayrs::FlatScene flat;
    std::vector<rayrs::SurfaceDev> surfaces;
    uint64_t n_objects = 0;
    int device = -1;
    ~rayrs_scene();
    rayrs::DevBuf d_prims, d_surfaces, d_hdri, d_counters;
    rayrs::DevBuf d_partial;
    rayrs::Event ev[3];
    hipStream_t last_stream = nullptr;
    bool pending = false;
    int cu_count = 0;
    struct Walk {
        rayrs::DevBuf d_nodes;
        int blocks_per_cu = 0;
        uint32_t stack_lds = 1;
        uint32_t hot_records = 0;
        uint32_t leafq = 0;
    };
    Walk trav[3];
    const rayrs::WalkTree& tree(int which) const { return which == 2 ? flat.gate_hot : which == 1 ? flat.gate : flat.walk; }
    rayrs::DevBuf d_hot;
    int walk_index(bool exact) const {
        if (!exact) return lab.gate_tree ? 1 : 0;
        return (flat.has_hot && lab.hot_group != 0xffffffffu) ? 2 : 1;
    }
    uint64_t device_bytes = 0;
    struct Pool {
        rayrs::DevBuf block;
        rayrs::DevBuf d_ctl;
        rayrs::DevBuf d_wave_items;
        rayrs::DevBuf d_stack_spill;
        rayrs::PinnedBuf h_live;
        rayrs::Event ev_batch[2];
        std::vector<rayrs::Event> ev_round;
        uint32_t timed_rounds = 0;
    };
    Pool pool;
    rayrs::DevBuf d_next_item;
    uint32_t rounds = 0;
    bool local_ok = false;
    bool last_local = false;
    bool last_exact = false;
    rayrs::LocalScene local = {};
    int local_blocks_per_cu = 1;
    rayrs::DevBuf d_local_light;
    rayrs::DevBuf d_local_items;
    rayrs::Stream multi_stream;
    rayrs::DevBuf multi_out;
    rayrs_tuning tuning = {};
    rayrs_lab_tuning lab = {};
};

namespace rayrs {
void set_last_error(const std::string& text);
int hip_fail(hipError_t e, const char* what);
int scene_upload(rayrs_scene* s);
SceneDev make_scene_dev(const rayrs_scene* s, bool exact);
CameraDev make_camera_dev(const rayrs_camera* c);
bool camera_is_far(const rayrs_scene* s, const rayrs_camera* c);
uint32_t trav_settings(const rayrs_scene* s, bool exact, uint32_t np, RenderDev& rp);
constexpr size_t POOL_SLOT_BYTES = sizeof(PathSlot) + 4 * sizeof(double) + 1u;
WfDev pool_wf(const DevBuf& block, uint32_t np, const DevBuf& ctl, uint32_t trav_blocks, const DevBuf& spill);
int render_enqueue(rayrs_scene* scene, const rayrs_camera* camera, const rayrs_render_params* params, uint32_t sample0,
                   const FilmPassDev* film, void* out_device, void* hip_stream);
}

#define HIP_TRY(expr)                                       \
    do {                                                    \
        hipError_t _e = (expr);                             \
        if (_e != hipSuccess) return rayrs::hip_fail(_e, #expr); \
    } while (0)

#define RAYRS_TRY(expr)                \
    do {                               \
        const int _s = (expr);         \
        if (_s != RAYRS_OK) return _s; \
    } while (0)

#define RAYRS_GUARDED(...)                                   \
    try {                                                    \
        __VA_ARGS__                                          \
    } catch (const std::bad_alloc&) {                        \
        rayrs::set_last_error("out of host memory");         \
        return RAYRS_OOM;                                    \
    } catch (const std::exception& e) {                      \
        rayrs::set_last_error(e.what());                     \
        return RAYRS_INVALID_ARG;                            \
    } catch (...) {                                          \
        rayrs::set_last_error("unknown exception");          \
        return RAYRS_INVALID_ARG;                            \
    }
```

### rayrs_amd/csrc/wavefront.h

```cpp
#pragma once
#include <hip/hip_runtime.h>

#include <cstddef>

#include "layout.h"

namespace rayrs {


struct RaySlot {
    double o[3];
    double d[3];
    double t;
    uint32_t prim;
    uint32_t bd;
};
static_assert(sizeof(RaySlot) == 64, "RaySlot");

struct TailSlot {
    double thr[3];
    double acc[3];
    uint32_t item;
    uint32_t s_cur;
    uint32_t s_end;
    uint32_t pix;
};
static_assert(sizeof(TailSlot) == 64, "TailSlot");

struct PathSlot {
    RaySlot ray;
    TailSlot tail;
};
static_assert(sizeof(PathSlot) == 128, "PathSlot");
constexpr uint32_t SLOT_ITEM_BIT = 1u << 31;
constexpr uint32_t SLOT_LIGHT_BIT = 1u << 30;
constexpr uint32_t SLOT_SAMPLE_MASK = (1u << 30) - 1u;

constexpr uint8_t WF_IDLE = 0;
constexpr uint8_t WF_READY = 1;
constexpr uint8_t WF_HIT = 2;
constexpr uint8_t WF_MISS = 3;
constexpr uint8_t WF_DEAD = 4;

struct alignas(128) WfCtl {
    uint32_t next_window;
    uint32_t pad0[31];
    uint32_t live_slots;
    uint32_t pad1[31];
};
static_assert(offsetof(WfCtl, live_slots) == 128 && sizeof(WfCtl) == 256, "WfCtl lines");

struct WfDev {
    PathSlot* slots;
    double* light;
    uint8_t* state;
    WfCtl* ctl;
    uint32_t np;
    unsigned long long* wave_items;
    uint32_t n_flat_waves;
    uint32_t trav_threads;
    uint32_t* stack_spill;
};

uint32_t wf_window_slots();
hipError_t wf_launch_init(const WfDev& wf, uint32_t live, hipStream_t stream);
hipError_t wf_launch_gen(bool compact, const SceneDev& sc, const CameraDev& cam, const RenderDev& rp, const WfDev& wf,
                         uint32_t blocks, hipStream_t stream);
hipError_t wf_launch_trav(bool compact, bool count, const SceneDev& sc, const RenderDev& rp, const WfDev& wf,
                          uint32_t blocks, hipStream_t stream);
uint32_t wf_trav_lds_bytes(bool compact, uint32_t stack_lds, uint32_t leafq, uint32_t hot_records);
hipError_t wf_trav_occupancy(bool compact, uint32_t lds, int* blocks_per_cu);
hipError_t wf_trav_raise_lds(bool compact, uint32_t lds);
hipError_t wf_launch_hit(bool compact, bool eager_light, const SceneDev& sc, const CameraDev& cam, const RenderDev& rp, const WfDev& wf,
                         uint32_t blocks, hipStream_t stream);
hipError_t wf_launch_miss(bool compact, bool eager_light, const SceneDev& sc, const CameraDev& cam, const RenderDev& rp, const WfDev& wf,
                          uint32_t blocks, hipStream_t stream);
hipError_t wf_launch_intake(const SceneDev& sc, const WfDev& wf, const double* o, const double* d, uint32_t n,
                            unsigned long long* answered, hipStream_t stream);

}
```

### rayrs_amd/csrc/wavefront.hip

```cpp
#include <hip/hip_runtime.h>

#include <map>
#include <mutex>

#include "device_path.h"
#include "kernels.h"
#include "lab_ticks.h"
#include "launch_dispatch.h"
#include "wavefront.h"

namespace rayrs {

constexpr uint32_t SPL = 8;
constexpr uint32_t WINDOW = 64 * SPL;
constexpr uint32_t HIT_SURFACES_LDS = 32;

static_assert(SPL == 8, "StateWords/BatchFeed assume two words per lane");
struct StateWords {
    uint32_t w[SPL / 4];
};

RR_DEV StateWords load_state_words(const WfDev& wf, uint32_t win) {
    const uint32_t* src = reinterpret_cast<const uint32_t*>(wf.state + win * WINDOW) + (threadIdx.x & 63u) * (SPL / 4);
    StateWords r;
#pragma unroll
    for (uint32_t k = 0; k < SPL / 4; k++) r.w[k] = src[k];
    return r;
}

RR_DEV uint32_t compact_words(const StateWords& sw, uint8_t want, uint16_t* list) {
    const uint32_t lane = threadIdx.x & 63u;
    const unsigned long long lanemask_lt = (1ull << lane) - 1ull;
    const uint32_t* words = sw.w;
    uint32_t count = 0;
#pragma unroll
    for (int j = 0; j < (int)SPL; j++) {
        const uint32_t s = (words[j >> 2] >> ((j & 3) * 8)) & 0xffu;
        const bool m = s == (uint32_t)want;
        const unsigned long long mask = __ballot(m);
        if (m) list[count + (uint32_t)__popcll(mask & lanemask_lt)] = (uint16_t)(lane * SPL + (uint32_t)j);
        count += (uint32_t)__popcll(mask);
    }
    return count;
}

RR_DEV uint32_t compact_window(const WfDev& wf, uint32_t win, uint8_t want, uint16_t* list) {
    return compact_words(load_state_words(wf, win), want, list);
}

RR_DEV uint8_t ready_state(V3 d) {
    const uint32_t key = (d.x < 0.0 ? 1u : 0u) | (d.y < 0.0 ? 2u : 0u) | (d.z < 0.0 ? 4u : 0u);
    return (uint8_t)(WF_READY | (key << 4));
}
RR_DEV uint32_t compact_window_ready(const WfDev& wf, uint32_t win, uint16_t* list) {
    const StateWords sw = load_state_words(wf, win);
    uint32_t count = 0;
#pragma nounroll
    for (uint32_t key = 0; key < 8u; key++) count += compact_words(sw, (uint8_t)(WF_READY | (key << 4)), list + count);
    return count;
}

RR_DEV uint8_t ready_state_pre(uint32_t mask) { return (uint8_t)(WF_READY | (mask << 3)); }
RR_DEV uint32_t compact_window_ready_pre(const WfDev& wf, uint32_t win, uint16_t* list) {
    const StateWords sw = load_state_words(wf, win);
    const uint32_t lane = threadIdx.x & 63u;
    const unsigned long long lanemask_lt = (1ull << lane) - 1ull;
    uint32_t count = 0;
#pragma nounroll
    for (uint32_t key = 0; key < 4u; key++) {
#pragma unroll
        for (int j = 0; j < (int)SPL; j++) {
            const uint32_t s = (sw.w[j >> 2] >> ((j & 3) * 8)) & 0xffu;
            const uint32_t m = (s >> 3) & 15u;
            const bool hit = (s & 7u) == (uint32_t)WF_READY && (m & (0u - m)) == (1u << key);
            const unsigned long long mask = __ballot(hit);
            if (hit) list[count + (uint32_t)__popcll(mask & lanemask_lt)] = (uint16_t)((lane * SPL + (uint32_t)j) | (m << 9));
            count += (uint32_t)__popcll(mask);
        }
    }
    return count;
}

constexpr uint32_t FEED_LIST = WINDOW + 64;

struct BatchFeed {
    uint32_t next_win, n_waves, n_windows, count, k, total;
    StateWords ahead;
    uint8_t want;
    uint32_t* list;
};

RR_DEV uint32_t compact_words_abs(const StateWords& sw, uint8_t want, uint32_t base, uint32_t* list) {
    const uint32_t lane = threadIdx.x & 63u;
    const uint32_t* words = sw.w;
    uint32_t count = 0;
#pragma unroll
    for (int j = 0; j < (int)SPL; j++) {
        const uint32_t s = (words[j >> 2] >> ((j & 3) * 8)) & 0xffu;
        const bool m = s == (uint32_t)want;
        const unsigned long long mask = __ballot(m);
        if (m) list[count + lanes_below(mask)] = base + lane * SPL + (uint32_t)j;
        count += (uint32_t)__popcll(mask);
    }
    return count;
}

RR_DEV void feed_init(BatchFeed& f, const WfDev& wf, uint32_t wave, uint32_t n_waves, uint8_t want, uint32_t* list) {
    f.next_win = wave, f.n_waves = n_waves, f.n_windows = wf.np / WINDOW;
    f.count = 0, f.k = 0, f.total = 0, f.want = want, f.list = list;
    f.ahead.w[0] = f.ahead.w[1] = 0;
    if (f.next_win < f.n_windows) f.ahead = load_state_words(wf, f.next_win);
}

RR_DEV bool feed_next(BatchFeed& f, const WfDev& wf, uint32_t& slot, bool& valid) {
    const uint32_t lane = threadIdx.x & 63u;
    while (f.count - f.k < 64u && f.next_win < f.n_windows) {
        const uint32_t left = f.count - f.k;
        const uint32_t carry = lane < left ? f.list[f.k + lane] : 0u;
        if (lane < left) f.list[lane] = carry;
        const uint32_t fresh = compact_words_abs(f.ahead, f.want, f.next_win * WINDOW, f.list + left);
        f.total += fresh;
        f.count = left + fresh;
        f.k = 0;
        f.next_win += f.n_waves;
        if (f.next_win < f.n_windows) f.ahead = load_state_words(wf, f.next_win);
    }
    if (f.k >= f.count) return false;
    valid = f.k + lane < f.count;
    slot = valid ? f.list[f.k + lane] : 0u;
    f.k += 64u;
    return true;
}

RR_DEV unsigned long long wave_sum(unsigned long long v) {
#pragma unroll
    for (int off = 32; off > 0; off >>= 1) {
        const uint32_t lo = (uint32_t)__shfl_xor((int)(uint32_t)v, off);
        const uint32_t hi = (uint32_t)__shfl_xor((int)(uint32_t)(v >> 32), off);
        v += ((unsigned long long)hi << 32) | lo;
    }
    return v;
}

RR_DEV void wave_atomic_add(unsigned long long* dst, unsigned long long v) {
    const unsigned long long s = wave_sum(v);
    if ((threadIdx.x & 63u) == 0 && s) atomicAdd(dst, s);
}

constexpr uint32_t ka_up(uint32_t off, uint32_t a) { return (off + a - 1u) / a * a; }
constexpr uint32_t KA_SC = 0;
constexpr uint32_t KA_CAM = ka_up(KA_SC + (uint32_t)sizeof(SceneDev), (uint32_t)alignof(CameraDev));
constexpr uint32_t KA_RP = ka_up(KA_CAM + (uint32_t)sizeof(CameraDev), (uint32_t)alignof(RenderDev));
constexpr uint32_t KA_WF = ka_up(KA_RP + (uint32_t)sizeof(RenderDev), (uint32_t)alignof(WfDev));
template <class T, uint32_t OFF>
RR_DEV const T& karg() {
    typedef const __attribute__((address_space(4))) char* KPtr;
    KPtr p = (KPtr)__builtin_amdgcn_kernarg_segment_ptr() + OFF;
    asm volatile("" : "+s"(p));
    return *(const T*)p;
}

RR_DEV RaySlot* ray_slot(const WfDev& wf, uint32_t slot) { return &wf.slots[slot].ray; }
RR_DEV TailSlot* tail_slot(const WfDev& wf, uint32_t slot) { return &wf.slots[slot].tail; }
RR_DEV double* light_slot(const WfDev& wf, uint32_t slot) { return wf.light + (size_t)slot * 4u; }


__global__ void __launch_bounds__(256) wf_init_kernel(WfDev wf, uint32_t live) {
    const uint32_t i = blockIdx.x * blockDim.x + threadIdx.x;
    if (i == 0) {
        WfCtl* c = wf.ctl;
        c->next_window = 0;
        c->live_slots = live;
    }
    if (i < 2u * wf.n_flat_waves) wf.wave_items[i] = 0ull;
    if (i >= wf.np) return;
    wf.state[i] = i < live ? WF_IDLE : WF_DEAD;
}


struct ItemRegs {
    double acc[3];
    uint32_t item, s_end, pix;
    uint32_t word;
    RR_DEV uint32_t cursor() const { return word & SLOT_SAMPLE_MASK; }
    RR_DEV bool has_item() const { return (word >> 31) != 0u; }
    RR_DEV bool has_light() const { return ((word >> 30) & 1u) != 0u; }
};

RR_DEV ItemRegs load_item(const WfDev& wf, uint32_t slot) {
    const TailSlot* t = tail_slot(wf, slot);
    ItemRegs r;
    r.acc[0] = t->acc[0], r.acc[1] = t->acc[1], r.acc[2] = t->acc[2];
    r.word = t->s_cur;
    r.item = t->item, r.s_end = t->s_end, r.pix = t->pix;
    return r;
}

RR_DEV uint64_t sample_key(const RenderDev& rp, const CameraDev& cam, const ItemRegs& ir) {
    return rr_path_key(rp.seed, (uint64_t)(ir.pix >> 16) * cam.W + (ir.pix & 0xffffu), (uint64_t)(ir.cursor() - 1u));
}

constexpr uint32_t ITEM_RESERVE = 256;
constexpr unsigned long long ITEMS_GONE = ~0ull;

struct ItemRange {
    unsigned long long next, end;
};

RR_DEV unsigned long long wave_uniform64(unsigned long long v) {
    const uint32_t lo = __builtin_amdgcn_readfirstlane((uint32_t)v), hi = __builtin_amdgcn_readfirstlane((uint32_t)(v >> 32));
    return ((unsigned long long)hi << 32) | lo;
}
template <bool SCALAR = false>
RR_DEV ItemRange load_item_range(const WfDev& wf, uint32_t wave) {
    ItemRange r;
    r.next = wf.wave_items[2 * (size_t)wave];
    r.end = wf.wave_items[2 * (size_t)wave + 1];
    if (SCALAR) r.next = wave_uniform64(r.next), r.end = wave_uniform64(r.end);
    return r;
}
RR_DEV void store_item_range(const WfDev& wf, uint32_t wave, const ItemRange& r) {
    if ((threadIdx.x & 63u) == 0) {
        wf.wave_items[2 * (size_t)wave] = r.next;
        wf.wave_items[2 * (size_t)wave + 1] = r.end;
    }
}

RR_DEV bool refill_item_range(const RenderDev& rp, ItemRange& range) {
    unsigned long long first = ITEMS_GONE;
    if (range.end != ITEMS_GONE) {
        if ((threadIdx.x & 63u) == 0) first = atomicAdd(rp.next_item, (unsigned long long)ITEM_RESERVE);
        const uint32_t flo = __builtin_amdgcn_readfirstlane((uint32_t)first);
        const uint32_t fhi = __builtin_amdgcn_readfirstlane((uint32_t)(first >> 32));
        first = ((unsigned long long)fhi << 32) | flo;
    }
    if (first >= rp.total_items) {
        range.next = range.end = ITEMS_GONE;
        return false;
    }
    range.next = first;
    range.end = first + ITEM_RESERVE < rp.total_items ? first + ITEM_RESERVE : rp.total_items;
    return true;
}

struct SampleCount {
    unsigned long long paths;
    unsigned long long direct;
// ... 149 lines not shown
    const uint32_t bd = nr.bd;
    const bool pre = karg<SceneDev, KA_SC>().hot != nullptr;
    if (__ballot(got) == 0ull) return;
    const bool primary = got && !carry;
    if (pre) {
        if (DEFER) {
            inv = mk(1.0 / d.x, 1.0 / d.y, 1.0 / d.z);
            enters = root_box_hit(karg<SceneDev, KA_SC>(), o, inv);
        }
        if (primary && !enters) sn.deferred++;
        finish_rays(got, enters, primary, slot, o, d, inv, bd, sn);
    } else if (got) {
        const WfDev& wf = karg<WfDev, KA_WF>();
        RaySlot* rs = ray_slot(wf, slot);
        rs->o[0] = o.x, rs->o[1] = o.y, rs->o[2] = o.z;
        rs->d[0] = d.x, rs->d[1] = d.y, rs->d[2] = d.z;
        rs->bd = bd;
        if (primary && !enters) {
            wf.state[slot] = WF_MISS;
            sn.deferred++;
        } else {
            wf.state[slot] = ready_state(d);
        }
    }
}

RR_DEV void store_sample_count(const SceneDev& sc, const RenderDev& rp, const WfDev& wf, const SampleCount& sn) {
    wave_atomic_add(&rp.counters->paths, sn.paths);
    const unsigned long long direct = wave_sum(sn.direct), deferred = wave_sum(sn.deferred);
    const unsigned long long pre = (unsigned long long)sn.pre_miss + sn.pre_done;
    if ((threadIdx.x & 63u) == 0 && (direct | deferred | pre)) {
        atomicAdd(&rp.counters->rays, direct + deferred + pre);
        if (direct) atomicAdd(&rp.counters->escaped_paths, direct);
        if (direct | deferred) atomicAdd(&rp.counters->direct_rays, direct + deferred);
    }
    if (rp.count_work && sc.hot != nullptr && (threadIdx.x & 63u) == 0) {
        Counters* c = rp.counters;
        const HotPtr h = hot_ptr(sc);
        const unsigned long long e = sn.hot.entered;
        atomicAdd(&c->pre_rays, pre);
        atomicAdd(&c->interior_visits, (unsigned long long)sn.pre_root);
        atomicAdd(&c->pre_root_records, (unsigned long long)sn.pre_root);
        atomicAdd(&c->hot_lane, (unsigned long long)sn.hot.owed);
        atomicAdd(&c->hot_prim_tests, e * h->count);
        atomicAdd(&c->hot_tri_divided, (unsigned long long)sn.hot.divided);
        if (h->n_tri) atomicAdd(&c->tri_tests, e * h->n_tri);
        if (h->n_sphere) atomicAdd(&c->sphere_tests, e * h->n_sphere);
        if (h->n_plane) atomicAdd(&c->plane_tests, e * h->n_plane);
    }
    const uint32_t r = (uint32_t)wave_sum(sn.retired);
    if ((threadIdx.x & 63u) == 0 && r) atomicSub(&wf.ctl->live_slots, r);
}

template <bool COMPACT>
__global__ void __launch_bounds__(256) wf_gen_kernel(SceneDev sc, CameraDev cam, RenderDev rp, WfDev wf) {
    __shared__ uint16_t lists[4][WINDOW];
    const uint32_t lane = threadIdx.x & 63u;
    uint16_t* list = lists[threadIdx.x >> 6];
    const uint32_t wave = (blockIdx.x * blockDim.x + threadIdx.x) >> 6;
    const uint32_t n_waves = (gridDim.x * blockDim.x) >> 6;
    const uint32_t n_windows = wf.np / WINDOW;
    SampleCount sn{0, 0, 0, 0, HotTally{0, 0, 0}, 0, 0, 0};
    ItemRange range = load_item_range(wf, wave);
    for (uint32_t win = wave; win < n_windows; win += n_waves) {
        const uint32_t count = compact_window(wf, win, WF_IDLE, list);
        for (uint32_t k = 0; k < count; k += 64u) {
            const bool valid = k + lane < count;
            const uint32_t slot = win * WINDOW + (valid ? (uint32_t)list[k + lane] : 0u);
            ItemRegs ir;
            ir.acc[0] = ir.acc[1] = ir.acc[2] = 0.0;
            ir.item = ir.s_end = ir.pix = ir.word = 0u;
            const NewRays nr = next_sample<COMPACT>(valid, slot, ir, false, range, sn);
            emit_rays<false>(slot, nr, sn);
        }
    }
    store_item_range(wf, wave, range);
    store_sample_count(sc, rp, wf, sn);
}



template <bool COMPACT, bool COUNT, bool EXACT, bool PRE>
__global__ void __launch_bounds__(256, 5) wf_trav_kernel(SceneDev sc, RenderDev rp, WfDev wf) {
    static_assert(EXACT || !PRE, "pre-tested rays are the default walk's");
    extern __shared__ uint32_t lds_dyn[];
    WfCtl* ctl = wf.ctl;
    if (ctl->live_slots == 0u) return;
    const uint32_t lane = threadIdx.x & 63u;
    const uint32_t wave = threadIdx.x >> 6;
    const uint32_t stack_words = (sc.stack_lds + 1u + sc.leafq) * 64u;
    const LaneStack stack{lds_dyn + (size_t)wave * stack_words + lane,
                          wf.stack_spill + ((size_t)blockIdx.x * 256u + threadIdx.x), sc.stack_lds, wf.trav_threads};
    uint16_t* list = reinterpret_cast<uint16_t*>(lds_dyn + 4u * (size_t)stack_words) + wave * WINDOW;
    uint4* hot_lds = reinterpret_cast<uint4*>(lds_dyn + 4u * (size_t)stack_words + 4u * WINDOW / 2u);
    {
        constexpr uint32_t G = COMPACT ? 8u : 16u;
        const uint4* src = reinterpret_cast<const uint4*>(sc.nodes);
        for (uint32_t i = threadIdx.x; i < sc.hot_records * G; i += 256u)
            hot_lds[(i / G) * HotNodes::stride<COMPACT>() + i % G] = src[i];
        __syncthreads();
    }
    const HotNodes hot{hot_lds, sc.hot_records};
    const unsigned long long lanemask_lt = (1ull << lane) - 1ull;
    uint32_t root_ref0 = 0, root_ref1 = 0, root_ref2 = 0, root_ref3 = 0;
    if (PRE) {
        const HotPtr h = hot_ptr(sc);
        root_ref0 = h->root_ref[0], root_ref1 = h->root_ref[1], root_ref2 = h->root_ref[2], root_ref3 = h->root_ref[3];
    }
    const uint32_t root_leaves = (root_ref0 >= REF_LEAF_BASE ? 1u : 0u) | (root_ref1 >= REF_LEAF_BASE ? 2u : 0u) |
                                 (root_ref2 >= REF_LEAF_BASE ? 4u : 0u) | (root_ref3 >= REF_LEAF_BASE ? 8u : 0u);

    const uint32_t n_windows = wf.np / WINDOW;
    const uint32_t n_waves = gridDim.x * 4u;
    const uint32_t static_windows = ctl->live_slots < wf.np / 4u ? n_windows : rp.static_windows;
    uint32_t static_next = blockIdx.x * 4u + wave;
    uint32_t list_pos = 0, list_len = 0, list_base = 0;
    bool no_more = false;

    bool active = false, pending = false;
    uint32_t slot = 0;
    V3 o = mk(0, 0, 0), d = mk(0, 0, 1);
    Trav tv;
    tv.inv = mk(0, 0, 0), tv.best_t = 0, tv.best_prim = 0xffffffffu, tv.cur = TRAV_DONE, tv.sp = 0;
    WorkCount wc{0, 0, 0, 0, 0};
    unsigned long long n_rays = 0;
    unsigned long long u_int_wave = 0, u_int_lane = 0, u_leaf_wave = 0, u_leaf_lane = 0;
    unsigned long long tk_int = 0, tk_leaf = 0, tk_refill = 0, tk_last = COUNT ? clock64() : 0ull;

    for (;;) {
        const bool at_int = EXACT ? (active && tv.cur != TRAV_DONE && defer_has_room(tv)) : (active && trav_at_interior(tv));
        const bool at_leaf = EXACT ? (active && defer_has_leaf(tv)) : (active && !trav_at_interior(tv));
        const int n_int = __popcll(__ballot(at_int));
        const int n_leaf = __popcll(__ballot(at_leaf));
        const int n_work = EXACT ? __popcll(__ballot(active)) : n_int + n_leaf;
        if ((n_work < (int)rp.refill_min && !no_more) || n_work == 0) {
            if (pending) {
                const bool hit = tv.best_prim != 0xffffffffu;
                if (hit) {
                    RaySlot* rs = ray_slot(wf, slot);
                    rs->t = tv.best_t;
                    rs->prim = tv.best_prim;
                }
                wf.state[slot] = hit ? WF_HIT : WF_MISS;
                pending = false;
            }
            if (no_more) break;
            bool need = !active;
            unsigned long long need_mask = __ballot(need);
            while (need_mask != 0ull) {
                if (list_pos >= list_len) {
                    uint32_t w = static_next;
                    if (w < static_windows) {
                        static_next += n_waves;
                    } else {
                        if (lane == 0) w = static_windows + atomicAdd(&ctl->next_window, 1u);
                        w = (uint32_t)__builtin_amdgcn_readfirstlane((int)w);
                    }
                    if (w >= n_windows) {
                        no_more = true;
                        break;
                    }
                    list_base = w * WINDOW;
                    list_len = PRE ? compact_window_ready_pre(wf, w, list) : compact_window_ready(wf, w, list);
                    list_pos = 0;
                    continue;
                }
                const uint32_t avail = list_len - list_pos;
                const uint32_t rank = (uint32_t)__popcll(need_mask & lanemask_lt);
                if (need && rank < avail) {
                    const uint32_t entry = (uint32_t)list[list_pos + rank];
                    slot = list_base + (PRE ? (entry & 511u) : entry);
                    const RaySlot* rs = ray_slot(wf, slot);
                    o = mk(rs->o[0], rs->o[1], rs->o[2]);
                    d = mk(rs->d[0], rs->d[1], rs->d[2]);
                    n_rays++;
                    if (PRE) {
                        tv.inv = mk(1.0 / d.x, 1.0 / d.y, 1.0 / d.z);
                        tv.best_t = rs->t;
                        tv.best_prim = rs->prim;
                        const uint32_t m = entry >> 9;
                        uint32_t r1 = root_ref1, r2 = root_ref2, r3 = root_ref3;
                        asm volatile("" : "+s"(r1), "+s"(r2), "+s"(r3));
                        const uint32_t mi = m & ~root_leaves, ml = m & root_leaves;
                        const int n = (int)__popc(mi);
                        const uint32_t low = mi & (0u - mi);
                        tv.cur = mi == 0u ? TRAV_DONE : (low & 1u) ? root_ref0 : (low & 2u) ? r1 : (low & 4u) ? r2 : r3;
                        tv.sp = n > 0 ? n - 1 : 0;
                        if ((mi & 2u) && low != 2u) stack.put(n - 1 - (int)__popc(mi & 1u), r1);
                        if ((mi & 4u) && low != 4u) stack.put(n - 1 - (int)__popc(mi & 3u), r2);
                        if ((mi & 8u) && low != 8u) stack.put(n - 1 - (int)__popc(mi & 7u), r3);
                        if (ml != 0u) {
                            if (ml & 1u) defer_take_ref(stack, tv, root_ref0);
                            if (ml & 2u) defer_take_ref(stack, tv, r1);
                            if (ml & 4u) defer_take_ref(stack, tv, r2);
                            if (ml & 8u) defer_take_ref(stack, tv, r3);
                        }
                        active = true;
                    } else {
                        trav_init(sc, o, d, tv);
                        if (tv.cur == TRAV_DONE) {
                            pending = true;
                        } else {
                            active = true;
                            if (EXACT && tv.cur >= REF_LEAF_BASE) {
                                const uint32_t ref = tv.cur;
                                tv.cur = TRAV_DONE;
                                defer_take_ref(stack, tv, ref);
                            }
                        }
                    }
                    need = false;
                }
                const uint32_t wanted = (uint32_t)__popcll(need_mask);
                list_pos += wanted < avail ? wanted : avail;
                need_mask = __ballot(need);
            }
            if (COUNT) {
                const unsigned long long now = clock64();
                tk_refill += now - tk_last, tk_last = now;
            }
            if (__ballot(active || pending) == 0ull && no_more) break;
            continue;
        }
        const bool leaf_phase = n_leaf >= (int)rp.leaf_min || n_int == 0 ||
                                (EXACT && __popcll(__ballot(at_leaf && !at_int)) >= (int)rp.leaf_wait);
        if (leaf_phase) {
            if (COUNT) u_leaf_wave += 1, u_leaf_lane += at_leaf ? 1 : 0;
            if (at_leaf) {
                if (EXACT) {
                    trav_leaf_step_defer<COMPACT, COUNT>(sc, o, d, stack, tv, wc);
                    if (defer_finished(tv)) active = false, pending = true;
                } else {
                    trav_leaf_step<COMPACT, COUNT>(sc, o, d, stack, tv, wc);
                    if (tv.cur == TRAV_DONE) active = false, pending = true;
                }
            }
            if (COUNT) {
                const unsigned long long now = clock64();
                tk_leaf += now - tk_last, tk_last = now;
            }
        } else {
            if (COUNT) u_int_wave += 1, u_int_lane += at_int ? 1 : 0;
            if (at_int) {
                if (EXACT) {
                    trav_interior_step_defer<COMPACT, COUNT>(sc, o, stack, hot, tv, wc);
                    if (defer_finished(tv)) active = false, pending = true;
                } else {
                    trav_interior_step<COMPACT, COUNT, false>(sc, o, stack, hot, tv, wc);
                    if (tv.cur == TRAV_DONE) active = false, pending = true;
                }
            }
            if (COUNT) {
                const unsigned long long now = clock64();
                tk_int += now - tk_last, tk_last = now;
            }
        }
    }

    Counters* c = rp.counters;
    wave_atomic_add(&c->rays, n_rays);
    if (COUNT) {
        wave_atomic_add(&c->interior_visits, wc.interior);
        wave_atomic_add(&c->tri_tests, wc.tri);
        wave_atomic_add(&c->sphere_tests, wc.sphere);
        wave_atomic_add(&c->plane_tests, wc.plane);
        wave_atomic_add(&c->step_wave, u_int_wave), wave_atomic_add(&c->step_lane, u_int_lane);
        wave_atomic_add(&c->inner_wave, u_leaf_lane), wave_atomic_add(&c->leaf_wave, u_leaf_wave);
        if (lane == 0) {
            atomicAdd(&c->interior_ticks, tk_int), atomicAdd(&c->leaf_ticks, tk_leaf);
            atomicAdd(&c->refill_ticks, tk_refill);
        }
    }
}


struct HitIn {
    uint32_t slot;
    bool valid;
    V3 o, d, thr, light;
    double t;
    uint32_t prim, bd;
    ItemRegs ir;
};

RR_DEV V3 load_light(const WfDev& wf, uint32_t slot) {
    const double* l = light_slot(wf, slot);
    return mk(l[0], l[1], l[2]);
}
RR_DEV bool light_is_plus_zero(V3 light) {
    return (rr_f64_bits(light.x) | rr_f64_bits(light.y) | rr_f64_bits(light.z)) == 0ull;
}

template <bool EAGER>
RR_DEV void load_hit_in(const WfDev& wf, HitIn& h) {
    const RaySlot* rs = ray_slot(wf, h.slot);
    h.o = mk(rs->o[0], rs->o[1], rs->o[2]);
    h.d = mk(rs->d[0], rs->d[1], rs->d[2]);
    h.t = rs->t;
    h.prim = rs->prim;
    h.bd = rs->bd;
    const TailSlot* t = tail_slot(wf, h.slot);
    h.thr = mk(t->thr[0], t->thr[1], t->thr[2]);
    h.light = EAGER ? load_light(wf, h.slot) : mk(0.0, 0.0, 0.0);
    h.ir = load_item(wf, h.slot);
}

template <bool COMPACT, bool EAGER>
__global__ void __launch_bounds__(256, 3) wf_hit_kernel(SceneDev sc, CameraDev cam, RenderDev rp, WfDev wf) {
    __shared__ uint32_t lists[4][FEED_LIST];
    __shared__ SurfaceDev s_surf[HIT_SURFACES_LDS];
    if (wf.ctl->live_slots == 0u) return;
    const uint32_t n_surf_lds = sc.n_surfaces < HIT_SURFACES_LDS ? sc.n_surfaces : HIT_SURFACES_LDS;
    for (uint32_t i = threadIdx.x; i < n_surf_lds * (uint32_t)(sizeof(SurfaceDev) / 4); i += 256u)
        reinterpret_cast<uint32_t*>(s_surf)[i] = reinterpret_cast<const uint32_t*>(sc.surfaces)[i];
    __syncthreads();
    uint32_t* list = lists[threadIdx.x >> 6];
    const uint32_t wave = (blockIdx.x * blockDim.x + threadIdx.x) >> 6;
    const uint32_t n_waves = (gridDim.x * blockDim.x) >> 6;
    SampleCount sn{0, 0, 0, 0, HotTally{0, 0, 0}, 0, 0, 0};
    if (blockIdx.x == 0 && threadIdx.x == 0) wf.ctl->next_window = 0;
    ItemRange range = load_item_range<true>(wf, wave);
    BatchFeed feed;
    feed_init(feed, wf, wave, n_waves, WF_HIT, list);
    HitIn cur;
    bool have = feed_next(feed, wf, cur.slot, cur.valid);
    PrimRec<COMPACT> rec_cur;
    if (have) {
        load_hit_in<EAGER>(wf, cur);
        rec_cur = load_prim<COMPACT>(sc.prims, cur.valid ? cur.prim : 0u);
    }
    RR_TICKS_BEGIN(7);
    while (have) {
        HitIn nxt;
        bool have_next = false;
        PrimRec<COMPACT> rec_nxt;
        {
            const uint32_t slot = cur.slot;
            const bool valid = cur.valid;
            bool ended = false, goes_on = false, acc_changed = false;
            uint32_t hit_sid = 8u;
            ItemRegs ir = cur.ir;
            V3 thr = mk(1.0, 1.0, 1.0), light = mk(0.0, 0.0, 0.0), position = mk(0.0, 0.0, 0.0), dir = mk(0.0, 0.0, 1.0);
            uint32_t bd_next = 0;
            if (valid) {
                RR_TICK_LOADS_ARRIVED(6)
                const SceneDev& sc = karg<SceneDev, KA_SC>();
                const RenderDev& rp = karg<RenderDev, KA_RP>();
                const WfDev& wf = karg<WfDev, KA_WF>();
                const V3 o = cur.o;
                const V3 d = cur.d;
                const double t = cur.t;
                const uint32_t bounce = cur.bd & 0xffffu;
                thr = bounce > 1u ? cur.thr : mk(1.0, 1.0, 1.0);
                light = mk(0.0, 0.0, 0.0);
                if (bounce > 1u && ir.has_light()) light = EAGER ? cur.light : load_light(wf, slot);
// ... 126 lines not shown
        ItemRegs ir = cur.ir;
        if (cur.valid) {
            const bool first = (cur.bd & 0xffffu) <= 1u;
            const V3 thr = first ? mk(1.0, 1.0, 1.0) : cur.thr;
            V3 light = mk(0.0, 0.0, 0.0);
            if (!first && ir.has_light()) light = EAGER ? cur.light : load_light(karg<WfDev, KA_WF>(), cur.slot);
            const V3 result = v_add(light, v_mul(thr, background(karg<SceneDev, KA_SC>(), cur.d)));
            ir.acc[0] += result.x;
            ir.acc[1] += result.y;
            ir.acc[2] += result.z;
        }
        RR_TICK(1)
        const NewRays nr = next_sample<COMPACT>(cur.valid, cur.slot, ir, true, range, sn);
        emit_rays<false>(cur.slot, nr, sn);
        RR_TICK(2)
        cur = nxt;
        have = have_next;
        RR_TICKS_BATCH();
    }
    RR_TICKS_END_MISS(rp)
    n_escaped = feed.total;
    store_item_range(wf, wave, range);
    if (lane == 0 && n_escaped) atomicAdd(&rp.counters->escaped_paths, n_escaped);
    store_sample_count(sc, rp, wf, sn);
}


__global__ void __launch_bounds__(256) wf_intake_kernel(SceneDev sc, CameraDev cam, RenderDev rp, WfDev wf, const double* o,
                                                        const double* d, uint32_t n, unsigned long long* answered) {
    const uint32_t slot = blockIdx.x * blockDim.x + threadIdx.x;
    const bool got = slot < n;
    const V3 ro = got ? mk(o[3 * slot], o[3 * slot + 1], o[3 * slot + 2]) : mk(0.0, 0.0, 0.0);
    const V3 rd = got ? mk(d[3 * slot], d[3 * slot + 1], d[3 * slot + 2]) : mk(0.0, 0.0, 1.0);
    const V3 inv = mk(1.0 / rd.x, 1.0 / rd.y, 1.0 / rd.z);
    const bool enters = got && root_box_hit(sc, ro, inv);
    if (sc.hot != nullptr) {
        SampleCount sn{0, 0, 0, 0, HotTally{0, 0, 0}, 0, 0, 0};
        finish_rays(got, enters, false, slot, ro, rd, inv, 1u, sn);
        if ((threadIdx.x & 63u) == 0 && sn.pre_done) atomicAdd(answered, (unsigned long long)sn.pre_done);
    } else if (got) {
        RaySlot* rs = ray_slot(wf, slot);
        rs->o[0] = ro.x, rs->o[1] = ro.y, rs->o[2] = ro.z;
        rs->d[0] = rd.x, rs->d[1] = rd.y, rs->d[2] = rd.z;
        rs->bd = 1u;
        wf.state[slot] = enters ? ready_state(rd) : WF_MISS;
    }
    if (!got && slot < wf.np) wf.state[slot] = WF_DEAD;
}


hipError_t wf_launch_intake(const SceneDev& sc, const WfDev& wf, const double* o, const double* d, uint32_t n,
                            unsigned long long* answered, hipStream_t stream) {
    const CameraDev cam{};
    const RenderDev rp{};
    hipLaunchKernelGGL(wf_intake_kernel, dim3(wf.np / 256u), dim3(256), 0, stream, sc, cam, rp, wf, o, d, n, answered);
    return hipGetLastError();
}

template <class F> struct ka_leading : std::false_type {};
template <class... Tail> struct ka_leading<void(SceneDev, CameraDev, RenderDev, WfDev, Tail...)> : std::true_type {};
static_assert(ka_leading<decltype(wf_gen_kernel<true>)>::value && ka_leading<decltype(wf_hit_kernel<true, true>)>::value &&
                  ka_leading<decltype(wf_miss_kernel<true, true>)>::value && ka_leading<decltype(wf_intake_kernel)>::value,
              "a kernel that calls karg() takes (SceneDev, CameraDev, RenderDev, WfDev) first");

uint32_t wf_trav_lds_bytes(bool compact, uint32_t stack_lds, uint32_t leafq, uint32_t hot_records) {
    return 4u * 64u * (stack_lds + 1u + leafq) * 4u + 4u * WINDOW * 2u + hot_records * (compact ? 144u : 272u);
}

uint32_t wf_window_slots() { return WINDOW; }

hipError_t wf_launch_init(const WfDev& wf, uint32_t live, hipStream_t stream) {
    hipLaunchKernelGGL(wf_init_kernel, dim3((wf.np + 255u) / 256u), dim3(256), 0, stream, wf, live);
    return hipGetLastError();
}

hipError_t wf_launch_gen(bool compact, const SceneDev& sc, const CameraDev& cam, const RenderDev& rp, const WfDev& wf,
                         uint32_t blocks, hipStream_t stream) {
    with_bools([&](auto C) {
        hipLaunchKernelGGL(wf_gen_kernel<C()>, dim3(blocks), dim3(256), 0, stream, sc, cam, rp, wf);
    }, compact);
    return hipGetLastError();
}

hipError_t wf_launch_trav(bool compact, bool count, const SceneDev& sc, const RenderDev& rp, const WfDev& wf,
                          uint32_t blocks, hipStream_t stream) {
    const uint32_t lds = wf_trav_lds_bytes(compact, sc.stack_lds, sc.leafq, sc.hot_records);
    with_bools([&](auto C, auto N, auto X, auto P) {
        hipLaunchKernelGGL((wf_trav_kernel<C(), N(), X(), X() && P()>), dim3(blocks), dim3(256), lds, stream, sc, rp, wf);
    }, compact, count, sc.exact != 0u, sc.hot != nullptr);
    return hipGetLastError();
}

hipError_t wf_trav_occupancy(bool compact, uint32_t lds, int* blocks_per_cu) {
    return with_bools([&](auto C) {
        return hipOccupancyMaxActiveBlocksPerMultiprocessor(blocks_per_cu, wf_trav_kernel<C(), false, false, false>, 256, lds);
    }, compact);
}

hipError_t wf_trav_raise_lds(bool compact, uint32_t lds) {
    static std::mutex mutex;
    static std::map<std::pair<int, bool>, uint32_t> raised;
    int device = 0;
    hipError_t e = hipGetDevice(&device);
    if (e != hipSuccess) return e;
    std::lock_guard<std::mutex> lock(mutex);
    uint32_t& set = raised[{device, compact}];
    if (lds <= set) return hipSuccess;
    e = with_bools([&](auto C) {
        const void* const instances[] = {
            reinterpret_cast<const void*>(&wf_trav_kernel<C(), false, false, false>), reinterpret_cast<const void*>(&wf_trav_kernel<C(), true, false, false>),
            reinterpret_cast<const void*>(&wf_trav_kernel<C(), false, true, false>), reinterpret_cast<const void*>(&wf_trav_kernel<C(), true, true, false>),
            reinterpret_cast<const void*>(&wf_trav_kernel<C(), false, true, true>), reinterpret_cast<const void*>(&wf_trav_kernel<C(), true, true, true>)};
        for (const void* k : instances) {
            const hipError_t ek = hipFuncSetAttribute(k, hipFuncAttributeMaxDynamicSharedMemorySize, (int)lds);
            if (ek != hipSuccess) return ek;
        }
        return hipSuccess;
    }, compact);
    if (e == hipSuccess) set = lds;
    return e;
}

hipError_t wf_launch_hit(bool compact, bool eager_light, const SceneDev& sc, const CameraDev& cam, const RenderDev& rp,
                         const WfDev& wf, uint32_t blocks, hipStream_t stream) {
    with_bools([&](auto C, auto E) {
        hipLaunchKernelGGL((wf_hit_kernel<C(), E()>), dim3(blocks), dim3(256), 0, stream, sc, cam, rp, wf);
    }, compact, eager_light);
    return hipGetLastError();
}

hipError_t wf_launch_miss(bool compact, bool eager_light, const SceneDev& sc, const CameraDev& cam, const RenderDev& rp,
                          const WfDev& wf, uint32_t blocks, hipStream_t stream) {
    with_bools([&](auto C, auto E) {
        hipLaunchKernelGGL((wf_miss_kernel<C(), E()>), dim3(blocks), dim3(256), 0, stream, sc, cam, rp, wf);
    }, compact, eager_light);
    return hipGetLastError();
}

}
```

Baseline: 5652.

## Add triangle-only specialized traversal kernel with batched vectorized triangle loads

Detects at build time whether every primitive outside the hot group is a triangle. When it is, a dedicated traversal kernel compiled with a TRI flag is used: leaf tests skip the per-primitive kind dispatch and read triangle records with wide uint4 loads, issuing two triangle loads together in compact mode. The shared traversal body moves into an include so it can be instantiated in both kernels. The new kernel also sets a launch-bounds occupancy hint, which may raise register pressure.

Result: faster. 5835, median of 6 (+3.2%).

```diff
diff --git a/include/rayrs_hip.h b/include/rayrs_hip.h
--- a/include/rayrs_hip.h
+++ b/include/rayrs_hip.h
@@ -109,7 +109,7 @@
     uint32_t hot_depth;
     uint32_t hot_first;
     uint32_t hot_count;
-    uint32_t hot_pad;
+    uint32_t hot_tri_only;
     double hot_box[6];
 } rayrs_scene_info_t;
 
@@ -173,7 +173,7 @@
     uint32_t local_pool;
     uint32_t exact_walk;
     uint32_t hot_group;
-    uint32_t stats_pad;
+    uint32_t tri_walk;
     uint64_t pre_rays;
     uint64_t pre_root_records;
     uint64_t hot_lane;
diff --git a/rayrs_amd/_ffi.py b/rayrs_amd/_ffi.py
--- a/rayrs_amd/_ffi.py
+++ b/rayrs_amd/_ffi.py
@@ -54,7 +54,7 @@
                 ("wide_depth", C.c_uint32), ("local_pool", C.c_uint32), ("gate_n_wide", C.c_uint32),
                 ("gate_root_ref", C.c_uint32), ("gate_depth", C.c_uint32),
                 ("hot_n_wide", C.c_uint32), ("hot_root_ref", C.c_uint32), ("hot_depth", C.c_uint32),
-                ("hot_first", C.c_uint32), ("hot_count", C.c_uint32), ("hot_pad", C.c_uint32),
+                ("hot_first", C.c_uint32), ("hot_count", C.c_uint32), ("hot_tri_only", C.c_uint32),
                 ("hot_box", C.c_double * 6)]
 
 
@@ -74,7 +74,7 @@
                 ("trace_ms", C.c_double), ("refill_ticks", C.c_uint64),
                 ("surface_hits", C.c_uint64 * 8), ("direct_rays", C.c_uint64), ("hit_ms", C.c_double), ("miss_ms", C.c_double),
                 ("local_pool", C.c_uint32), ("exact_walk", C.c_uint32), ("hot_group", C.c_uint32),
-                ("stats_pad", C.c_uint32), ("pre_rays", C.c_uint64), ("pre_root_records", C.c_uint64), ("hot_lane", C.c_uint64),
+                ("tri_walk", C.c_uint32), ("pre_rays", C.c_uint64), ("pre_root_records", C.c_uint64), ("hot_lane", C.c_uint64),
                 ("hot_prim_tests", C.c_uint64), ("hot_tri_divided", C.c_uint64)]
 
     def as_dict(self):
diff --git a/rayrs_amd/csrc/abi.cpp b/rayrs_amd/csrc/abi.cpp
--- a/rayrs_amd/csrc/abi.cpp
+++ b/rayrs_amd/csrc/abi.cpp
@@ -323,6 +323,7 @@
         info->hot_depth = f.gate_hot.depth;
         info->hot_first = f.hot.first;
         info->hot_count = f.hot.count;
+        info->hot_tri_only = f.hot_tri_only ? 1u : 0u;
         for (int i = 0; i < 6; i++) info->hot_box[i] = f.hot.box[i];
     }
     info->local_pool = (scene->local_ok && scene->tuning.local_pool != 1u) ? 1u : 0u;
@@ -497,7 +498,7 @@
     RAYRS_FIELD(rayrs_scene_info_t, gate_depth);
     RAYRS_FIELD(rayrs_scene_info_t, hot_n_wide), RAYRS_FIELD(rayrs_scene_info_t, hot_root_ref);
     RAYRS_FIELD(rayrs_scene_info_t, hot_depth), RAYRS_FIELD(rayrs_scene_info_t, hot_first);
-    RAYRS_FIELD(rayrs_scene_info_t, hot_count), RAYRS_FIELD(rayrs_scene_info_t, hot_pad);
+    RAYRS_FIELD(rayrs_scene_info_t, hot_count), RAYRS_FIELD(rayrs_scene_info_t, hot_tri_only);
     RAYRS_FIELD(rayrs_scene_info_t, hot_box);
     RAYRS_STRUCT(rayrs_render_params, 9);
     RAYRS_FIELD(rayrs_render_params, spp), RAYRS_FIELD(rayrs_render_params, max_bounces);
@@ -519,7 +520,7 @@
     RAYRS_FIELD(rayrs_render_stats, surface_hits), RAYRS_FIELD(rayrs_render_stats, direct_rays);
     RAYRS_FIELD(rayrs_render_stats, hit_ms), RAYRS_FIELD(rayrs_render_stats, miss_ms);
     RAYRS_FIELD(rayrs_render_stats, local_pool), RAYRS_FIELD(rayrs_render_stats, exact_walk);
-    RAYRS_FIELD(rayrs_render_stats, hot_group), RAYRS_FIELD(rayrs_render_stats, stats_pad);
+    RAYRS_FIELD(rayrs_render_stats, hot_group), RAYRS_FIELD(rayrs_render_stats, tri_walk);
     RAYRS_FIELD(rayrs_render_stats, pre_rays), RAYRS_FIELD(rayrs_render_stats, pre_root_records);
     RAYRS_FIELD(rayrs_render_stats, hot_lane);
     RAYRS_FIELD(rayrs_render_stats, hot_prim_tests), RAYRS_FIELD(rayrs_render_stats, hot_tri_divided);
@@ -574,6 +575,7 @@
     sc.t0 = s->flat.t0;
     sc.t1 = s->flat.t1;
     sc.exact = exact ? 1u : 0u;
+    sc.tri_only = (which == 2 && s->flat.hot_tri_only) ? 1u : 0u;
     return sc;
 }
 
@@ -830,6 +832,7 @@
     p.is_film = film != nullptr;
     p.film = film ? *film : FilmPassDev{};
     scene->last_exact = p.exact;
+    scene->last_tri = wf_trav_is_tri(p.sc);
 
     rayrs_scene::Pool& pl = scene->pool;
     HIP_TRY(scene->d_partial.reserve((size_t)p.partial_need * 3 * sizeof(double)));
@@ -913,6 +916,7 @@
         stats->local_pool = scene->last_local ? 1u : 0u;
         stats->exact_walk = (scene->last_exact || scene->last_local) ? 1u : 0u;
         stats->hot_group = (!scene->last_local && scene->last_exact && scene->walk_index(true) == 2) ? 1u : 0u;
+        stats->tri_walk = (!scene->last_local && scene->last_tri) ? 1u : 0u;
         stats->kernel_launches = (uint64_t)scene->rounds;
     }
     return RAYRS_OK;
diff --git a/rayrs_amd/csrc/device_path.h b/rayrs_amd/csrc/device_path.h
--- a/rayrs_amd/csrc/device_path.h
+++ b/rayrs_amd/csrc/device_path.h
@@ -557,6 +557,80 @@
                 tv.best_prim = p;
             }
         }
+    }
+}
+
+template <bool COMPACT>
+struct TriRec {
+    uint4 q[COMPACT ? 2 : 4];
+    uint32_t lo, hi;
+    RR_DEV uint32_t dw(int i) const {
+        if (i == (COMPACT ? 8 : 16)) return lo;
+        if (i == (COMPACT ? 9 : 17)) return hi;
+        const uint4& v = q[i >> 2];
+        switch (i & 3) {
+            case 0: return v.x;
+            case 1: return v.y;
+            case 2: return v.z;
+            default: return v.w;
+        }
+    }
+    RR_DEV double coord(int i) const {
+        if (COMPACT) return (double)__uint_as_float(dw(i));
+        return f64_from(dw(2 * i), dw(2 * i + 1));
+    }
+};
+
+template <bool COMPACT>
+RR_DEV TriRec<COMPACT> load_tri(const void* prims, uint32_t p) {
+    TriRec<COMPACT> r;
+    const uint4* src = reinterpret_cast<const uint4*>(prims) + (size_t)p * (COMPACT ? 3 : 5);
+#pragma unroll
+    for (int i = 0; i < (COMPACT ? 2 : 4); i++) r.q[i] = src[i];
+    if (COMPACT) {
+        r.lo = reinterpret_cast<const uint32_t*>(src)[8];
+        r.hi = 0u;
+    } else {
+        const uint2 t = reinterpret_cast<const uint2*>(src)[8];
+        r.lo = t.x, r.hi = t.y;
+    }
+    return r;
+}
+
+template <bool COMPACT>
+RR_DEV void tri_rec_test(const SceneDev& sc, const TriRec<COMPACT>& r, uint32_t p, V3 o, V3 d, Trav& tv) {
+    const V3 p1 = mk(r.coord(0), r.coord(1), r.coord(2));
+    const V3 p2 = mk(r.coord(3), r.coord(4), r.coord(5));
+    const V3 p3 = mk(r.coord(6), r.coord(7), r.coord(8));
+    double t;
+    if (triangle_intersect(p1, p2, p3, o, d, t) && t > sc.t0 && t < sc.t1) {
+        if (t < tv.best_t || (t == tv.best_t && p < tv.best_prim)) {
+            tv.best_t = t;
+            tv.best_prim = p;
+        }
+    }
+}
+
+template <bool COMPACT, bool COUNT>
+RR_DEV void trav_leaf_step_defer_tri(const SceneDev& sc, V3 o, V3 d, const LaneStack& stack, Trav& tv, WorkCount& wc) {
+    tv.sp -= (int)LEAFQ_ONE;
+    const uint32_t ref = defer_queue(stack)[((uint32_t)tv.sp >> 16) * 64u];
+    const uint32_t first = (ref & 0x3fffffffu) >> 2;
+    const uint32_t count = (ref & 3u) + 1u;
+    if (COUNT) wc.leaf_prims = count, wc.tri += count;
+    if (COMPACT) {
+        for (uint32_t k = 0; k < count; k += 2u) {
+            const uint32_t p = first + k;
+            const bool two = k + 1u < count;
+            const TriRec<COMPACT> ra = load_tri<COMPACT>(sc.prims, p);
+            TriRec<COMPACT> rb;
+            if (two) rb = load_tri<COMPACT>(sc.prims, p + 1u);
+            __builtin_amdgcn_sched_barrier(0);
+            tri_rec_test<COMPACT>(sc, ra, p, o, d, tv);
+            if (two) tri_rec_test<COMPACT>(sc, rb, p + 1u, o, d, tv);
+        }
+    } else {
+        for (uint32_t k = 0; k < count; k++) tri_rec_test<COMPACT>(sc, load_tri<COMPACT>(sc.prims, first + k), first + k, o, d, tv);
     }
 }
 
diff --git a/rayrs_amd/csrc/layout.h b/rayrs_amd/csrc/layout.h
--- a/rayrs_amd/csrc/layout.h
+++ b/rayrs_amd/csrc/layout.h
@@ -89,7 +89,8 @@
     double root_box[6];
     double t0, t1;
     double hdri_wm1, hdri_hm1;
-    uint32_t exact, pad1;
+    uint32_t exact;
+    uint32_t tri_only;
     const HotGroupDev* hot;
 };
 
diff --git a/rayrs_amd/csrc/scene_host.cpp b/rayrs_amd/csrc/scene_host.cpp
--- a/rayrs_amd/csrc/scene_host.cpp
+++ b/rayrs_amd/csrc/scene_host.cpp
@@ -749,6 +749,11 @@
             else if (s.kind == PRIM_PLANE) f.hot.n_plane++;
             else f.hot.n_tri++;
         }
+        f.hot_tri_only = true;
+        for (size_t p = 0; p < n && f.hot_tri_only; p++) {
+            if (p >= f.hot.first && p < (size_t)f.hot.first + f.hot.count) continue;
+            if (objs.objs[f.prim_object[p]].geom.kind != PRIM_TRIANGLE) f.hot_tri_only = false;
+        }
         const WalkTree& t = f.gate_hot;
         const uint32_t r = t.root_ref & 0x3fffffffu;
         const double inf = std::numeric_limits<double>::infinity();
diff --git a/rayrs_amd/csrc/scene_host.hpp b/rayrs_amd/csrc/scene_host.hpp
--- a/rayrs_amd/csrc/scene_host.hpp
+++ b/rayrs_amd/csrc/scene_host.hpp
@@ -56,6 +56,7 @@
     uint32_t depth = 0;
     WalkTree walk, gate, gate_hot;
     bool has_hot = false;
+    bool hot_tri_only = false;
     HotGroupDev hot = {};
     double root_box[6] = {0, 0, 0, 0, 0, 0};
     bool compact = false;
diff --git a/rayrs_amd/csrc/scene_internal.hpp b/rayrs_amd/csrc/scene_internal.hpp
--- a/rayrs_amd/csrc/scene_internal.hpp
+++ b/rayrs_amd/csrc/scene_internal.hpp
@@ -59,6 +59,7 @@
     uint32_t rounds = 0;
     bool local_ok = false;
     bool last_local = false;
+    bool last_tri = false;
     bool last_exact = false;
     rayrs::LocalScene local = {};
     int local_blocks_per_cu = 1;
diff --git a/rayrs_amd/csrc/wavefront.h b/rayrs_amd/csrc/wavefront.h
--- a/rayrs_amd/csrc/wavefront.h
+++ b/rayrs_amd/csrc/wavefront.h
@@ -69,6 +69,11 @@
 hipError_t wf_launch_trav(bool compact, bool count, const SceneDev& sc, const RenderDev& rp, const WfDev& wf,
                           uint32_t blocks, hipStream_t stream);
 uint32_t wf_trav_lds_bytes(bool compact, uint32_t stack_lds, uint32_t leafq, uint32_t hot_records);
+bool wf_trav_is_tri(const SceneDev& sc);
+hipError_t wf_launch_trav_tri(bool compact, bool count, uint32_t lds, const SceneDev& sc, const RenderDev& rp, const WfDev& wf,
+                              uint32_t blocks, hipStream_t stream);
+hipError_t wf_trav_tri_occupancy(bool compact, uint32_t lds, int* blocks_per_cu);
+hipError_t wf_trav_tri_raise_lds(bool compact, uint32_t lds);
 hipError_t wf_trav_occupancy(bool compact, uint32_t lds, int* blocks_per_cu);
 hipError_t wf_trav_raise_lds(bool compact, uint32_t lds);
 hipError_t wf_launch_hit(bool compact, bool eager_light, const SceneDev& sc, const CameraDev& cam, const RenderDev& rp, const WfDev& wf,
diff --git a/rayrs_amd/csrc/wavefront.hip b/rayrs_amd/csrc/wavefront.hip
--- a/rayrs_amd/csrc/wavefront.hip
+++ b/rayrs_amd/csrc/wavefront.hip
@@ -8,161 +8,9 @@
 #include "lab_ticks.h"
 #include "launch_dispatch.h"
 #include "wavefront.h"
+#include "wavefront_dev.h"
 
 namespace rayrs {
-
-constexpr uint32_t SPL = 8;
-constexpr uint32_t WINDOW = 64 * SPL;
-constexpr uint32_t HIT_SURFACES_LDS = 32;
-
-static_assert(SPL == 8, "StateWords/BatchFeed assume two words per lane");
-struct StateWords {
-    uint32_t w[SPL / 4];
-};
-
-RR_DEV StateWords load_state_words(const WfDev& wf, uint32_t win) {
-    const uint32_t* src = reinterpret_cast<const uint32_t*>(wf.state + win * WINDOW) + (threadIdx.x & 63u) * (SPL / 4);
-    StateWords r;
-#pragma unroll
-    for (uint32_t k = 0; k < SPL / 4; k++) r.w[k] = src[k];
-    return r;
-}
-
-RR_DEV uint32_t compact_words(const StateWords& sw, uint8_t want, uint16_t* list) {
-    const uint32_t lane = threadIdx.x & 63u;
-    const unsigned long long lanemask_lt = (1ull << lane) - 1ull;
-    const uint32_t* words = sw.w;
-    uint32_t count = 0;
-#pragma unroll
-    for (int j = 0; j < (int)SPL; j++) {
-        const uint32_t s = (words[j >> 2] >> ((j & 3) * 8)) & 0xffu;
-        const bool m = s == (uint32_t)want;
-        const unsigned long long mask = __ballot(m);
-        if (m) list[count + (uint32_t)__popcll(mask & lanemask_lt)] = (uint16_t)(lane * SPL + (uint32_t)j);
-        count += (uint32_t)__popcll(mask);
-    }
-    return count;
-}
-
-RR_DEV uint32_t compact_window(const WfDev& wf, uint32_t win, uint8_t want, uint16_t* list) {
-    return compact_words(load_state_words(wf, win), want, list);
-}
-
-RR_DEV uint8_t ready_state(V3 d) {
-    const uint32_t key = (d.x < 0.0 ? 1u : 0u) | (d.y < 0.0 ? 2u : 0u) | (d.z < 0.0 ? 4u : 0u);
-    return (uint8_t)(WF_READY | (key << 4));
-}
-RR_DEV uint32_t compact_window_ready(const WfDev& wf, uint32_t win, uint16_t* list) {
-    const StateWords sw = load_state_words(wf, win);
-    uint32_t count = 0;
-#pragma nounroll
-    for (uint32_t key = 0; key < 8u; key++) count += compact_words(sw, (uint8_t)(WF_READY | (key << 4)), list + count);
-    return count;
-}
-
-RR_DEV uint8_t ready_state_pre(uint32_t mask) { return (uint8_t)(WF_READY | (mask << 3)); }
-RR_DEV uint32_t compact_window_ready_pre(const WfDev& wf, uint32_t win, uint16_t* list) {
-    const StateWords sw = load_state_words(wf, win);
-    const uint32_t lane = threadIdx.x & 63u;
-    const unsigned long long lanemask_lt = (1ull << lane) - 1ull;
-    uint32_t count = 0;
-#pragma nounroll
-    for (uint32_t key = 0; key < 4u; key++) {
-#pragma unroll
-        for (int j = 0; j < (int)SPL; j++) {
-            const uint32_t s = (sw.w[j >> 2] >> ((j & 3) * 8)) & 0xffu;
-            const uint32_t m = (s >> 3) & 15u;
-            const bool hit = (s & 7u) == (uint32_t)WF_READY && (m & (0u - m)) == (1u << key);
-            const unsigned long long mask = __ballot(hit);
-            if (hit) list[count + (uint32_t)__popcll(mask & lanemask_lt)] = (uint16_t)((lane * SPL + (uint32_t)j) | (m << 9));
-            count += (uint32_t)__popcll(mask);
-        }
-    }
-    return count;
-}
-
-constexpr uint32_t FEED_LIST = WINDOW + 64;
-
-struct BatchFeed {
-    uint32_t next_win, n_waves, n_windows, count, k, total;
-    StateWords ahead;
-    uint8_t want;
-    uint32_t* list;
-};
-
-RR_DEV uint32_t compact_words_abs(const StateWords& sw, uint8_t want, uint32_t base, uint32_t* list) {
-    const uint32_t lane = threadIdx.x & 63u;
-    const uint32_t* words = sw.w;
-    uint32_t count = 0;
-#pragma unroll
-    for (int j = 0; j < (int)SPL; j++) {
-        const uint32_t s = (words[j >> 2] >> ((j & 3) * 8)) & 0xffu;
-        const bool m = s == (uint32_t)want;
-        const unsigned long long mask = __ballot(m);
-        if (m) list[count + lanes_below(mask)] = base + lane * SPL + (uint32_t)j;
-        count += (uint32_t)__popcll(mask);
-    }
-    return count;
-}
-
-RR_DEV void feed_init(BatchFeed& f, const WfDev& wf, uint32_t wave, uint32_t n_waves, uint8_t want, uint32_t* list) {
-    f.next_win = wave, f.n_waves = n_waves, f.n_windows = wf.np / WINDOW;
-    f.count = 0, f.k = 0, f.total = 0, f.want = want, f.list = list;
-    f.ahead.w[0] = f.ahead.w[1] = 0;
-    if (f.next_win < f.n_windows) f.ahead = load_state_words(wf, f.next_win);
-}
-
-RR_DEV bool feed_next(BatchFeed& f, const WfDev& wf, uint32_t& slot, bool& valid) {
-    const uint32_t lane = threadIdx.x & 63u;
-    while (f.count - f.k < 64u && f.next_win < f.n_windows) {
-        const uint32_t left = f.count - f.k;
-        const uint32_t carry = lane < left ? f.list[f.k + lane] : 0u;
-        if (lane < left) f.list[lane] = carry;
-        const uint32_t fresh = compact_words_abs(f.ahead, f.want, f.next_win * WINDOW, f.list + left);
-        f.total += fresh;
-        f.count = left + fresh;
-        f.k = 0;
-        f.next_win += f.n_waves;
-        if (f.next_win < f.n_windows) f.ahead = load_state_words(wf, f.next_win);
-    }
-    if (f.k >= f.count) return false;
-    valid = f.k + lane < f.count;
-    slot = valid ? f.list[f.k + lane] : 0u;
-    f.k += 64u;
-    return true;
-}
-
-RR_DEV unsigned long long wave_sum(unsigned long long v) {
-#pragma unroll
-    for (int off = 32; off > 0; off >>= 1) {
-        const uint32_t lo = (uint32_t)__shfl_xor((int)(uint32_t)v, off);
-        const uint32_t hi = (uint32_t)__shfl_xor((int)(uint32_t)(v >> 32), off);
-        v += ((unsigned long long)hi << 32) | lo;
-    }
-    return v;
-}
-
-RR_DEV void wave_atomic_add(unsigned long long* dst, unsigned long long v) {
-    const unsigned long long s = wave_sum(v);
-    if ((threadIdx.x & 63u) == 0 && s) atomicAdd(dst, s);
-}
-
-constexpr uint32_t ka_up(uint32_t off, uint32_t a) { return (off + a - 1u) / a * a; }
-constexpr uint32_t KA_SC = 0;
-constexpr uint32_t KA_CAM = ka_up(KA_SC + (uint32_t)sizeof(SceneDev), (uint32_t)alignof(CameraDev));
-constexpr uint32_t KA_RP = ka_up(KA_CAM + (uint32_t)sizeof(CameraDev), (uint32_t)alignof(RenderDev));
-constexpr uint32_t KA_WF = ka_up(KA_RP + (uint32_t)sizeof(RenderDev), (uint32_t)alignof(WfDev));
-template <class T, uint32_t OFF>
-RR_DEV const T& karg() {
-    typedef const __attribute__((address_space(4))) char* KPtr;
-    KPtr p = (KPtr)__builtin_amdgcn_kernarg_segment_ptr() + OFF;
-    asm volatile("" : "+s"(p));
-    return *(const T*)p;
-}
-
-RR_DEV RaySlot* ray_slot(const WfDev& wf, uint32_t slot) { return &wf.slots[slot].ray; }
-RR_DEV TailSlot* tail_slot(const WfDev& wf, uint32_t slot) { return &wf.slots[slot].tail; }
-RR_DEV double* light_slot(const WfDev& wf, uint32_t slot) { return wf.light + (size_t)slot * 4u; }
 
 
 __global__ void __launch_bounds__(256) wf_init_kernel(WfDev wf, uint32_t live) {
@@ -478,195 +326,8 @@
 
 template <bool COMPACT, bool COUNT, bool EXACT, bool PRE>
 __global__ void __launch_bounds__(256, 5) wf_trav_kernel(SceneDev sc, RenderDev rp, WfDev wf) {
-    static_assert(EXACT || !PRE, "pre-tested rays are the default walk's");
-    extern __shared__ uint32_t lds_dyn[];
-    WfCtl* ctl = wf.ctl;
-    if (ctl->live_slots == 0u) return;
-    const uint32_t lane = threadIdx.x & 63u;
-    const uint32_t wave = threadIdx.x >> 6;
-    const uint32_t stack_words = (sc.stack_lds + 1u + sc.leafq) * 64u;
-    const LaneStack stack{lds_dyn + (size_t)wave * stack_words + lane,
-                          wf.stack_spill + ((size_t)blockIdx.x * 256u + threadIdx.x), sc.stack_lds, wf.trav_threads};
-    uint16_t* list = reinterpret_cast<uint16_t*>(lds_dyn + 4u * (size_t)stack_words) + wave * WINDOW;
-    uint4* hot_lds = reinterpret_cast<uint4*>(lds_dyn + 4u * (size_t)stack_words + 4u * WINDOW / 2u);
-    {
-        constexpr uint32_t G = COMPACT ? 8u : 16u;
-        const uint4* src = reinterpret_cast<const uint4*>(sc.nodes);
-        for (uint32_t i = threadIdx.x; i < sc.hot_records * G; i += 256u)
-            hot_lds[(i / G) * HotNodes::stride<COMPACT>() + i % G] = src[i];
-        __syncthreads();
-    }
-    const HotNodes hot{hot_lds, sc.hot_records};
-    const unsigned long long lanemask_lt = (1ull << lane) - 1ull;
-    uint32_t root_ref0 = 0, root_ref1 = 0, root_ref2 = 0, root_ref3 = 0;
-    if (PRE) {
-        const HotPtr h = hot_ptr(sc);
-        root_ref0 = h->root_ref[0], root_ref1 = h->root_ref[1], root_ref2 = h->root_ref[2], root_ref3 = h->root_ref[3];
-    }
-    const uint32_t root_leaves = (root_ref0 >= REF_LEAF_BASE ? 1u : 0u) | (root_ref1 >= REF_LEAF_BASE ? 2u : 0u) |
-                                 (root_ref2 >= REF_LEAF_BASE ? 4u : 0u) | (root_ref3 >= REF_LEAF_BASE ? 8u : 0u);
-
-    const uint32_t n_windows = wf.np / WINDOW;
-    const uint32_t n_waves = gridDim.x * 4u;
-    const uint32_t static_windows = ctl->live_slots < wf.np / 4u ? n_windows : rp.static_windows;
-    uint32_t static_next = blockIdx.x * 4u + wave;
-    uint32_t list_pos = 0, list_len = 0, list_base = 0;
-    bool no_more = false;
-
-    bool active = false, pending = false;
-    uint32_t slot = 0;
-    V3 o = mk(0, 0, 0), d = mk(0, 0, 1);
-    Trav tv;
-    tv.inv = mk(0, 0, 0), tv.best_t = 0, tv.best_prim = 0xffffffffu, tv.cur = TRAV_DONE, tv.sp = 0;
-    WorkCount wc{0, 0, 0, 0, 0};
-    unsigned long long n_rays = 0;
-    unsigned long long u_int_wave = 0, u_int_lane = 0, u_leaf_wave = 0, u_leaf_lane = 0;
-    unsigned long long tk_int = 0, tk_leaf = 0, tk_refill = 0, tk_last = COUNT ? clock64() : 0ull;
-
-    for (;;) {
-        const bool at_int = EXACT ? (active && tv.cur != TRAV_DONE && defer_has_room(tv)) : (active && trav_at_interior(tv));
-        const bool at_leaf = EXACT ? (active && defer_has_leaf(tv)) : (active && !trav_at_interior(tv));
-        const int n_int = __popcll(__ballot(at_int));
-        const int n_leaf = __popcll(__ballot(at_leaf));
-        const int n_work = EXACT ? __popcll(__ballot(active)) : n_int + n_leaf;
-        if ((n_work < (int)rp.refill_min && !no_more) || n_work == 0) {
-            if (pending) {
-                const bool hit = tv.best_prim != 0xffffffffu;
-                if (hit) {
-                    RaySlot* rs = ray_slot(wf, slot);
-                    rs->t = tv.best_t;
-                    rs->prim = tv.best_prim;
-                }
-                wf.state[slot] = hit ? WF_HIT : WF_MISS;
-                pending = false;
-            }
-            if (no_more) break;
-            bool need = !active;
-            unsigned long long need_mask = __ballot(need);
-            while (need_mask != 0ull) {
-                if (list_pos >= list_len) {
-                    uint32_t w = static_next;
-                    if (w < static_windows) {
-                        static_next += n_waves;
-                    } else {
-                        if (lane == 0) w = static_windows + atomicAdd(&ctl->next_window, 1u);
-                        w = (uint32_t)__builtin_amdgcn_readfirstlane((int)w);
-                    }
-                    if (w >= n_windows) {
-                        no_more = true;
-                        break;
-                    }
-                    list_base = w * WINDOW;
-                    list_len = PRE ? compact_window_ready_pre(wf, w, list) : compact_window_ready(wf, w, list);
-                    list_pos = 0;
-                    continue;
-                }
-                const uint32_t avail = list_len - list_pos;
-                const uint32_t rank = (uint32_t)__popcll(need_mask & lanemask_lt);
-                if (need && rank < avail) {
-                    const uint32_t entry = (uint32_t)list[list_pos + rank];
-                    slot = list_base + (PRE ? (entry & 511u) : entry);
-                    const RaySlot* rs = ray_slot(wf, slot);
-                    o = mk(rs->o[0], rs->o[1], rs->o[2]);
-                    d = mk(rs->d[0], rs->d[1], rs->d[2]);
-                    n_rays++;
-                    if (PRE) {
-                        tv.inv = mk(1.0 / d.x, 1.0 / d.y, 1.0 / d.z);
-                        tv.best_t = rs->t;
-                        tv.best_prim = rs->prim;
-                        const uint32_t m = entry >> 9;
-                        uint32_t r1 = root_ref1, r2 = root_ref2, r3 = root_ref3;
-                        asm volatile("" : "+s"(r1), "+s"(r2), "+s"(r3));
-                        const uint32_t mi = m & ~root_leaves, ml = m & root_leaves;
-                        const int n = (int)__popc(mi);
-                        const uint32_t low = mi & (0u - mi);
-                        tv.cur = mi == 0u ? TRAV_DONE : (low & 1u) ? root_ref0 : (low & 2u) ? r1 : (low & 4u) ? r2 : r3;
-                        tv.sp = n > 0 ? n - 1 : 0;
-                        if ((mi & 2u) && low != 2u) stack.put(n - 1 - (int)__popc(mi & 1u), r1);
-                        if ((mi & 4u) && low != 4u) stack.put(n - 1 - (int)__popc(mi & 3u), r2);
-                        if ((mi & 8u) && low != 8u) stack.put(n - 1 - (int)__popc(mi & 7u), r3);
-                        if (ml != 0u) {
-                            if (ml & 1u) defer_take_ref(stack, tv, root_ref0);
-                            if (ml & 2u) defer_take_ref(stack, tv, r1);
-                            if (ml & 4u) defer_take_ref(stack, tv, r2);
-                            if (ml & 8u) defer_take_ref(stack, tv, r3);
-                        }
-                        active = true;
-                    } else {
-                        trav_init(sc, o, d, tv);
-                        if (tv.cur == TRAV_DONE) {
-                            pending = true;
-                        } else {
-                            active = true;
-                            if (EXACT && tv.cur >= REF_LEAF_BASE) {
-                                const uint32_t ref = tv.cur;
-                                tv.cur = TRAV_DONE;
-                                defer_take_ref(stack, tv, ref);
-                            }
-                        }
-                    }
-                    need = false;
-                }
-                const uint32_t wanted = (uint32_t)__popcll(need_mask);
-                list_pos += wanted < avail ? wanted : avail;
-                need_mask = __ballot(need);
-            }
-            if (COUNT) {
-                const unsigned long long now = clock64();
-                tk_refill += now - tk_last, tk_last = now;
-            }
-            if (__ballot(active || pending) == 0ull && no_more) break;
-            continue;
-        }
-        const bool leaf_phase = n_leaf >= (int)rp.leaf_min || n_int == 0 ||
-                                (EXACT && __popcll(__ballot(at_leaf && !at_int)) >= (int)rp.leaf_wait);
-        if (leaf_phase) {
-            if (COUNT) u_leaf_wave += 1, u_leaf_lane += at_leaf ? 1 : 0;
-            if (at_leaf) {
-                if (EXACT) {
-                    trav_leaf_step_defer<COMPACT, COUNT>(sc, o, d, stack, tv, wc);
-                    if (defer_finished(tv)) active = false, pending = true;
-                } else {
-                    trav_leaf_step<COMPACT, COUNT>(sc, o, d, stack, tv, wc);
-                    if (tv.cur == TRAV_DONE) active = false, pending = true;
-                }
-            }
-            if (COUNT) {
-                const unsigned long long now = clock64();
-                tk_leaf += now - tk_last, tk_last = now;
-            }
-        } else {
-            if (COUNT) u_int_wave += 1, u_int_lane += at_int ? 1 : 0;
-            if (at_int) {
-                if (EXACT) {
-                    trav_interior_step_defer<COMPACT, COUNT>(sc, o, stack, hot, tv, wc);
-                    if (defer_finished(tv)) active = false, pending = true;
-                } else {
-                    trav_interior_step<COMPACT, COUNT, false>(sc, o, stack, hot, tv, wc);
-                    if (tv.cur == TRAV_DONE) active = false, pending = true;
-                }
-            }
-            if (COUNT) {
-                const unsigned long long now = clock64();
-                tk_int += now - tk_last, tk_last = now;
-            }
-        }
-    }
-
-    Counters* c = rp.counters;
-    wave_atomic_add(&c->rays, n_rays);
-    if (COUNT) {
-        wave_atomic_add(&c->interior_visits, wc.interior);
-        wave_atomic_add(&c->tri_tests, wc.tri);
-        wave_atomic_add(&c->sphere_tests, wc.sphere);
-        wave_atomic_add(&c->plane_tests, wc.plane);
-        wave_atomic_add(&c->step_wave, u_int_wave), wave_atomic_add(&c->step_lane, u_int_lane);
-        wave_atomic_add(&c->inner_wave, u_leaf_lane), wave_atomic_add(&c->leaf_wave, u_leaf_wave);
-        if (lane == 0) {
-            atomicAdd(&c->interior_ticks, tk_int), atomicAdd(&c->leaf_ticks, tk_leaf);
-            atomicAdd(&c->refill_ticks, tk_refill);
-        }
-    }
+    constexpr bool TRI = false;
+#include "wavefront_trav_body.h"
 }
 
 
@@ -959,9 +620,12 @@
     return hipGetLastError();
 }
 
+bool wf_trav_is_tri(const SceneDev& sc) { return sc.tri_only != 0u && sc.exact != 0u && sc.hot != nullptr; }
+
 hipError_t wf_launch_trav(bool compact, bool count, const SceneDev& sc, const RenderDev& rp, const WfDev& wf,
                           uint32_t blocks, hipStream_t stream) {
     const uint32_t lds = wf_trav_lds_bytes(compact, sc.stack_lds, sc.leafq, sc.hot_records);
+    if (wf_trav_is_tri(sc)) return wf_launch_trav_tri(compact, count, lds, sc, rp, wf, blocks, stream);
     with_bools([&](auto C, auto N, auto X, auto P) {
         hipLaunchKernelGGL((wf_trav_kernel<C(), N(), X(), X() && P()>), dim3(blocks), dim3(256), lds, stream, sc, rp, wf);
     }, compact, count, sc.exact != 0u, sc.hot != nullptr);
@@ -970,7 +634,12 @@
 
 hipError_t wf_trav_occupancy(bool compact, uint32_t lds, int* blocks_per_cu) {
     return with_bools([&](auto C) {
-        return hipOccupancyMaxActiveBlocksPerMultiprocessor(blocks_per_cu, wf_trav_kernel<C(), false, false, false>, 256, lds);
+        int tri = 0;
+        hipError_t e = hipOccupancyMaxActiveBlocksPerMultiprocessor(blocks_per_cu, wf_trav_kernel<C(), false, false, false>, 256, lds);
+        if (e != hipSuccess) return e;
+        e = wf_trav_tri_occupancy(C(), lds, &tri);
+        if (e == hipSuccess && tri < *blocks_per_cu) *blocks_per_cu = tri;
+        return e;
     }, compact);
 }
 
@@ -992,7 +661,7 @@
             const hipError_t ek = hipFuncSetAttribute(k, hipFuncAttributeMaxDynamicSharedMemorySize, (int)lds);
             if (ek != hipSuccess) return ek;
         }
-        return hipSuccess;
+        return wf_trav_tri_raise_lds(C(), lds);
     }, compact);
     if (e == hipSuccess) set = lds;
     return e;
@@ -1014,4 +683,5 @@
     return hipGetLastError();
 }
 
-}
+
+}
diff --git a/rayrs_amd/csrc/wavefront_dev.h b/rayrs_amd/csrc/wavefront_dev.h
--- /dev/null
+++ b/rayrs_amd/csrc/wavefront_dev.h
@@ -0,0 +1,162 @@
+#pragma once
+#include <hip/hip_runtime.h>
+
+#include "device_path.h"
+#include "wavefront.h"
+
+namespace rayrs {
+
+constexpr uint32_t SPL = 8;
+constexpr uint32_t WINDOW = 64 * SPL;
+constexpr uint32_t HIT_SURFACES_LDS = 32;
+
+static_assert(SPL == 8, "StateWords/BatchFeed assume two words per lane");
+struct StateWords {
+    uint32_t w[SPL / 4];
+};
+
+RR_DEV StateWords load_state_words(const WfDev& wf, uint32_t win) {
+    const uint32_t* src = reinterpret_cast<const uint32_t*>(wf.state + win * WINDOW) + (threadIdx.x & 63u) * (SPL / 4);
+    StateWords r;
+#pragma unroll
+    for (uint32_t k = 0; k < SPL / 4; k++) r.w[k] = src[k];
+    return r;
+}
+
+RR_DEV uint32_t compact_words(const StateWords& sw, uint8_t want, uint16_t* list) {
+    const uint32_t lane = threadIdx.x & 63u;
+    const unsigned long long lanemask_lt = (1ull << lane) - 1ull;
+    const uint32_t* words = sw.w;
+    uint32_t count = 0;
+#pragma unroll
+    for (int j = 0; j < (int)SPL; j++) {
+        const uint32_t s = (words[j >> 2] >> ((j & 3) * 8)) & 0xffu;
+        const bool m = s == (uint32_t)want;
+        const unsigned long long mask = __ballot(m);
+        if (m) list[count + (uint32_t)__popcll(mask & lanemask_lt)] = (uint16_t)(lane * SPL + (uint32_t)j);
+        count += (uint32_t)__popcll(mask);
+    }
+    return count;
+}
+
+RR_DEV uint32_t compact_window(const WfDev& wf, uint32_t win, uint8_t want, uint16_t* list) {
+    return compact_words(load_state_words(wf, win), want, list);
+}
+
+RR_DEV uint8_t ready_state(V3 d) {
+    const uint32_t key = (d.x < 0.0 ? 1u : 0u) | (d.y < 0.0 ? 2u : 0u) | (d.z < 0.0 ? 4u : 0u);
+    return (uint8_t)(WF_READY | (key << 4));
+}
+RR_DEV uint32_t compact_window_ready(const WfDev& wf, uint32_t win, uint16_t* list) {
+    const StateWords sw = load_state_words(wf, win);
+    uint32_t count = 0;
+#pragma nounroll
+    for (uint32_t key = 0; key < 8u; key++) count += compact_words(sw, (uint8_t)(WF_READY | (key << 4)), list + count);
+    return count;
+}
+
+RR_DEV uint8_t ready_state_pre(uint32_t mask) { return (uint8_t)(WF_READY | (mask << 3)); }
+RR_DEV uint32_t compact_window_ready_pre(const WfDev& wf, uint32_t win, uint16_t* list) {
+    const StateWords sw = load_state_words(wf, win);
+    const uint32_t lane = threadIdx.x & 63u;
+    const unsigned long long lanemask_lt = (1ull << lane) - 1ull;
+    uint32_t count = 0;
+#pragma nounroll
+    for (uint32_t key = 0; key < 4u; key++) {
+#pragma unroll
+        for (int j = 0; j < (int)SPL; j++) {
+            const uint32_t s = (sw.w[j >> 2] >> ((j & 3) * 8)) & 0xffu;
+            const uint32_t m = (s >> 3) & 15u;
+            const bool hit = (s & 7u) == (uint32_t)WF_READY && (m & (0u - m)) == (1u << key);
+            const unsigned long long mask = __ballot(hit);
+            if (hit) list[count + (uint32_t)__popcll(mask & lanemask_lt)] = (uint16_t)((lane * SPL + (uint32_t)j) | (m << 9));
+            count += (uint32_t)__popcll(mask);
+        }
+    }
+    return count;
+}
+
+constexpr uint32_t FEED_LIST = WINDOW + 64;
+
+struct BatchFeed {
+    uint32_t next_win, n_waves, n_windows, count, k, total;
+    StateWords ahead;
+    uint8_t want;
+    uint32_t* list;
+};
+
+RR_DEV uint32_t compact_words_abs(const StateWords& sw, uint8_t want, uint32_t base, uint32_t* list) {
+    const uint32_t lane = threadIdx.x & 63u;
+    const uint32_t* words = sw.w;
+    uint32_t count = 0;
+#pragma unroll
+    for (int j = 0; j < (int)SPL; j++) {
+        const uint32_t s = (words[j >> 2] >> ((j & 3) * 8)) & 0xffu;
+        const bool m = s == (uint32_t)want;
+        const unsigned long long mask = __ballot(m);
+        if (m) list[count + lanes_below(mask)] = base + lane * SPL + (uint32_t)j;
+        count += (uint32_t)__popcll(mask);
+    }
+    return count;
+}
+
+RR_DEV void feed_init(BatchFeed& f, const WfDev& wf, uint32_t wave, uint32_t n_waves, uint8_t want, uint32_t* list) {
+    f.next_win = wave, f.n_waves = n_waves, f.n_windows = wf.np / WINDOW;
+    f.count = 0, f.k = 0, f.total = 0, f.want = want, f.list = list;
+    f.ahead.w[0] = f.ahead.w[1] = 0;
+    if (f.next_win < f.n_windows) f.ahead = load_state_words(wf, f.next_win);
+}
+
+RR_DEV bool feed_next(BatchFeed& f, const WfDev& wf, uint32_t& slot, bool& valid) {
+    const uint32_t lane = threadIdx.x & 63u;
+    while (f.count - f.k < 64u && f.next_win < f.n_windows) {
+        const uint32_t left = f.count - f.k;
+        const uint32_t carry = lane < left ? f.list[f.k + lane] : 0u;
+        if (lane < left) f.list[lane] = carry;
+        const uint32_t fresh = compact_words_abs(f.ahead, f.want, f.next_win * WINDOW, f.list + left);
+        f.total += fresh;
+        f.count = left + fresh;
+        f.k = 0;
+        f.next_win += f.n_waves;
+        if (f.next_win < f.n_windows) f.ahead = load_state_words(wf, f.next_win);
+    }
+    if (f.k >= f.count) return false;
+    valid = f.k + lane < f.count;
+    slot = valid ? f.list[f.k + lane] : 0u;
+    f.k += 64u;
+    return true;
+}
+
+RR_DEV unsigned long long wave_sum(unsigned long long v) {
+#pragma unroll
+    for (int off = 32; off > 0; off >>= 1) {
+        const uint32_t lo = (uint32_t)__shfl_xor((int)(uint32_t)v, off);
+        const uint32_t hi = (uint32_t)__shfl_xor((int)(uint32_t)(v >> 32), off);
+        v += ((unsigned long long)hi << 32) | lo;
+    }
+    return v;
+}
+
+RR_DEV void wave_atomic_add(unsigned long long* dst, unsigned long long v) {
+    const unsigned long long s = wave_sum(v);
+    if ((threadIdx.x & 63u) == 0 && s) atomicAdd(dst, s);
+}
+
+constexpr uint32_t ka_up(uint32_t off, uint32_t a) { return (off + a - 1u) / a * a; }
+constexpr uint32_t KA_SC = 0;
+constexpr uint32_t KA_CAM = ka_up(KA_SC + (uint32_t)sizeof(SceneDev), (uint32_t)alignof(CameraDev));
+constexpr uint32_t KA_RP = ka_up(KA_CAM + (uint32_t)sizeof(CameraDev), (uint32_t)alignof(RenderDev));
+constexpr uint32_t KA_WF = ka_up(KA_RP + (uint32_t)sizeof(RenderDev), (uint32_t)alignof(WfDev));
+template <class T, uint32_t OFF>
+RR_DEV const T& karg() {
+    typedef const __attribute__((address_space(4))) char* KPtr;
+    KPtr p = (KPtr)__builtin_amdgcn_kernarg_segment_ptr() + OFF;
+    asm volatile("" : "+s"(p));
+    return *(const T*)p;
+}
+
+RR_DEV RaySlot* ray_slot(const WfDev& wf, uint32_t slot) { return &wf.slots[slot].ray; }
+RR_DEV TailSlot* tail_slot(const WfDev& wf, uint32_t slot) { return &wf.slots[slot].tail; }
+RR_DEV double* light_slot(const WfDev& wf, uint32_t slot) { return wf.light + (size_t)slot * 4u; }
+
+}
diff --git a/rayrs_amd/csrc/wavefront_trav_body.h b/rayrs_amd/csrc/wavefront_trav_body.h
--- /dev/null
+++ b/rayrs_amd/csrc/wavefront_trav_body.h
@@ -0,0 +1,190 @@
+    static_assert(EXACT || !PRE, "pre-tested rays are the default walk's");
+    extern __shared__ uint32_t lds_dyn[];
+    WfCtl* ctl = wf.ctl;
+    if (ctl->live_slots == 0u) return;
+    const uint32_t lane = threadIdx.x & 63u;
+    const uint32_t wave = threadIdx.x >> 6;
+    const uint32_t stack_words = (sc.stack_lds + 1u + sc.leafq) * 64u;
+    const LaneStack stack{lds_dyn + (size_t)wave * stack_words + lane,
+                          wf.stack_spill + ((size_t)blockIdx.x * 256u + threadIdx.x), sc.stack_lds, wf.trav_threads};
+    uint16_t* list = reinterpret_cast<uint16_t*>(lds_dyn + 4u * (size_t)stack_words) + wave * WINDOW;
+    uint4* hot_lds = reinterpret_cast<uint4*>(lds_dyn + 4u * (size_t)stack_words + 4u * WINDOW / 2u);
+    {
+        constexpr uint32_t G = COMPACT ? 8u : 16u;
+        const uint4* src = reinterpret_cast<const uint4*>(sc.nodes);
+        for (uint32_t i = threadIdx.x; i < sc.hot_records * G; i += 256u)
+            hot_lds[(i / G) * HotNodes::stride<COMPACT>() + i % G] = src[i];
+        __syncthreads();
+    }
+    const HotNodes hot{hot_lds, sc.hot_records};
+    const unsigned long long lanemask_lt = (1ull << lane) - 1ull;
+    uint32_t root_ref0 = 0, root_ref1 = 0, root_ref2 = 0, root_ref3 = 0;
+    if (PRE) {
+        const HotPtr h = hot_ptr(sc);
+        root_ref0 = h->root_ref[0], root_ref1 = h->root_ref[1], root_ref2 = h->root_ref[2], root_ref3 = h->root_ref[3];
+    }
+    const uint32_t root_leaves = (root_ref0 >= REF_LEAF_BASE ? 1u : 0u) | (root_ref1 >= REF_LEAF_BASE ? 2u : 0u) |
+                                 (root_ref2 >= REF_LEAF_BASE ? 4u : 0u) | (root_ref3 >= REF_LEAF_BASE ? 8u : 0u);
+
+    const uint32_t n_windows = wf.np / WINDOW;
+    const uint32_t n_waves = gridDim.x * 4u;
+    const uint32_t static_windows = ctl->live_slots < wf.np / 4u ? n_windows : rp.static_windows;
+    uint32_t static_next = blockIdx.x * 4u + wave;
+    uint32_t list_pos = 0, list_len = 0, list_base = 0;
+    bool no_more = false;
+
+    bool active = false, pending = false;
+    uint32_t slot = 0;
+    V3 o = mk(0, 0, 0), d = mk(0, 0, 1);
+    Trav tv;
+    tv.inv = mk(0, 0, 0), tv.best_t = 0, tv.best_prim = 0xffffffffu, tv.cur = TRAV_DONE, tv.sp = 0;
+    WorkCount wc{0, 0, 0, 0, 0};
+    unsigned long long n_rays = 0;
+    unsigned long long u_int_wave = 0, u_int_lane = 0, u_leaf_wave = 0, u_leaf_lane = 0;
+    unsigned long long tk_int = 0, tk_leaf = 0, tk_refill = 0, tk_last = COUNT ? clock64() : 0ull;
+
+    for (;;) {
+        const bool at_int = EXACT ? (active && tv.cur != TRAV_DONE && defer_has_room(tv)) : (active && trav_at_interior(tv));
+        const bool at_leaf = EXACT ? (active && defer_has_leaf(tv)) : (active && !trav_at_interior(tv));
+        const int n_int = __popcll(__ballot(at_int));
+        const int n_leaf = __popcll(__ballot(at_leaf));
+        const int n_work = EXACT ? __popcll(__ballot(active)) : n_int + n_leaf;
+        if ((n_work < (int)rp.refill_min && !no_more) || n_work == 0) {
+            if (pending) {
+                const bool hit = tv.best_prim != 0xffffffffu;
+                if (hit) {
+                    RaySlot* rs = ray_slot(wf, slot);
+                    rs->t = tv.best_t;
+                    rs->prim = tv.best_prim;
+                }
+                wf.state[slot] = hit ? WF_HIT : WF_MISS;
+                pending = false;
+            }
+            if (no_more) break;
+            bool need = !active;
+            unsigned long long need_mask = __ballot(need);
+            while (need_mask != 0ull) {
+                if (list_pos >= list_len) {
+                    uint32_t w = static_next;
+                    if (w < static_windows) {
+                        static_next += n_waves;
+                    } else {
+                        if (lane == 0) w = static_windows + atomicAdd(&ctl->next_window, 1u);
+                        w = (uint32_t)__builtin_amdgcn_readfirstlane((int)w);
+                    }
+                    if (w >= n_windows) {
+                        no_more = true;
+                        break;
+                    }
+                    list_base = w * WINDOW;
+                    list_len = PRE ? compact_window_ready_pre(wf, w, list) : compact_window_ready(wf, w, list);
+                    list_pos = 0;
+                    continue;
+                }
+                const uint32_t avail = list_len - list_pos;
+                const uint32_t rank = (uint32_t)__popcll(need_mask & lanemask_lt);
+                if (need && rank < avail) {
+                    const uint32_t entry = (uint32_t)list[list_pos + rank];
+                    slot = list_base + (PRE ? (entry & 511u) : entry);
+                    const RaySlot* rs = ray_slot(wf, slot);
+                    o = mk(rs->o[0], rs->o[1], rs->o[2]);
+                    d = mk(rs->d[0], rs->d[1], rs->d[2]);
+                    n_rays++;
+                    if (PRE) {
+                        tv.inv = mk(1.0 / d.x, 1.0 / d.y, 1.0 / d.z);
+                        tv.best_t = rs->t;
+                        tv.best_prim = rs->prim;
+                        const uint32_t m = entry >> 9;
+                        uint32_t r1 = root_ref1, r2 = root_ref2, r3 = root_ref3;
+                        asm volatile("" : "+s"(r1), "+s"(r2), "+s"(r3));
+                        const uint32_t mi = m & ~root_leaves, ml = m & root_leaves;
+                        const int n = (int)__popc(mi);
+                        const uint32_t low = mi & (0u - mi);
+                        tv.cur = mi == 0u ? TRAV_DONE : (low & 1u) ? root_ref0 : (low & 2u) ? r1 : (low & 4u) ? r2 : r3;
+                        tv.sp = n > 0 ? n - 1 : 0;
+                        if ((mi & 2u) && low != 2u) stack.put(n - 1 - (int)__popc(mi & 1u), r1);
+                        if ((mi & 4u) && low != 4u) stack.put(n - 1 - (int)__popc(mi & 3u), r2);
+                        if ((mi & 8u) && low != 8u) stack.put(n - 1 - (int)__popc(mi & 7u), r3);
+                        if (ml != 0u) {
+                            if (ml & 1u) defer_take_ref(stack, tv, root_ref0);
+                            if (ml & 2u) defer_take_ref(stack, tv, r1);
+                            if (ml & 4u) defer_take_ref(stack, tv, r2);
+                            if (ml & 8u) defer_take_ref(stack, tv, r3);
+                        }
+                        active = true;
+                    } else {
+                        trav_init(sc, o, d, tv);
+                        if (tv.cur == TRAV_DONE) {
+                            pending = true;
+                        } else {
+                            active = true;
+                            if (EXACT && tv.cur >= REF_LEAF_BASE) {
+                                const uint32_t ref = tv.cur;
+                                tv.cur = TRAV_DONE;
+                                defer_take_ref(stack, tv, ref);
+                            }
+                        }
+                    }
+                    need = false;
+                }
+                const uint32_t wanted = (uint32_t)__popcll(need_mask);
+                list_pos += wanted < avail ? wanted : avail;
+                need_mask = __ballot(need);
+            }
+            if (COUNT) {
+                const unsigned long long now = clock64();
+                tk_refill += now - tk_last, tk_last = now;
+            }
+            if (__ballot(active || pending) == 0ull && no_more) break;
+            continue;
+        }
+        const bool leaf_phase = n_leaf >= (int)rp.leaf_min || n_int == 0 ||
+                                (EXACT && __popcll(__ballot(at_leaf && !at_int)) >= (int)rp.leaf_wait);
+        if (leaf_phase) {
+            if (COUNT) u_leaf_wave += 1, u_leaf_lane += at_leaf ? 1 : 0;
+            if (at_leaf) {
+                if (EXACT) {
+                    if (TRI) trav_leaf_step_defer_tri<COMPACT, COUNT>(sc, o, d, stack, tv, wc);
+                    else trav_leaf_step_defer<COMPACT, COUNT>(sc, o, d, stack, tv, wc);
+                    if (defer_finished(tv)) active = false, pending = true;
+                } else {
+                    trav_leaf_step<COMPACT, COUNT>(sc, o, d, stack, tv, wc);
+                    if (tv.cur == TRAV_DONE) active = false, pending = true;
+                }
+            }
+            if (COUNT) {
+                const unsigned long long now = clock64();
+                tk_leaf += now - tk_last, tk_last = now;
+            }
+        } else {
+            if (COUNT) u_int_wave += 1, u_int_lane += at_int ? 1 : 0;
+            if (at_int) {
+                if (EXACT) {
+                    trav_interior_step_defer<COMPACT, COUNT>(sc, o, stack, hot, tv, wc);
+                    if (defer_finished(tv)) active = false, pending = true;
+                } else {
+                    trav_interior_step<COMPACT, COUNT, false>(sc, o, stack, hot, tv, wc);
+                    if (tv.cur == TRAV_DONE) active = false, pending = true;
+                }
+            }
+            if (COUNT) {
+                const unsigned long long now = clock64();
+                tk_int += now - tk_last, tk_last = now;
+            }
+        }
+    }
+
+    Counters* c = rp.counters;
+    wave_atomic_add(&c->rays, n_rays);
+    if (COUNT) {
+        wave_atomic_add(&c->interior_visits, wc.interior);
+        wave_atomic_add(&c->tri_tests, wc.tri);
+        wave_atomic_add(&c->sphere_tests, wc.sphere);
+        wave_atomic_add(&c->plane_tests, wc.plane);
+        wave_atomic_add(&c->step_wave, u_int_wave), wave_atomic_add(&c->step_lane, u_int_lane);
+        wave_atomic_add(&c->inner_wave, u_leaf_lane), wave_atomic_add(&c->leaf_wave, u_leaf_wave);
+        if (lane == 0) {
+            atomicAdd(&c->interior_ticks, tk_int), atomicAdd(&c->leaf_ticks, tk_leaf);
+            atomicAdd(&c->refill_ticks, tk_refill);
+        }
+    }
diff --git a/rayrs_amd/csrc/wavefront_tri.hip b/rayrs_amd/csrc/wavefront_tri.hip
--- /dev/null
+++ b/rayrs_amd/csrc/wavefront_tri.hip
@@ -0,0 +1,40 @@
+#include <hip/hip_runtime.h>
+
+#include "device_path.h"
+#include "launch_dispatch.h"
+#include "wavefront.h"
+#include "wavefront_dev.h"
+
+namespace rayrs {
+
+template <bool COMPACT, bool COUNT>
+__global__ void __launch_bounds__(256, 5) wf_trav_tri_kernel(SceneDev sc, RenderDev rp, WfDev wf) {
+    constexpr bool TRI = true, EXACT = true, PRE = true;
+#include "wavefront_trav_body.h"
+}
+
+hipError_t wf_launch_trav_tri(bool compact, bool count, uint32_t lds, const SceneDev& sc, const RenderDev& rp, const WfDev& wf,
+                              uint32_t blocks, hipStream_t stream) {
+    with_bools([&](auto C, auto N) {
+        hipLaunchKernelGGL((wf_trav_tri_kernel<C(), N()>), dim3(blocks), dim3(256), lds, stream, sc, rp, wf);
+    }, compact, count);
+    return hipGetLastError();
+}
+
+hipError_t wf_trav_tri_occupancy(bool compact, uint32_t lds, int* blocks_per_cu) {
+    return with_bools([&](auto C) {
+        return hipOccupancyMaxActiveBlocksPerMultiprocessor(blocks_per_cu, wf_trav_tri_kernel<C(), false>, 256, lds);
+    }, compact);
+}
+
+hipError_t wf_trav_tri_raise_lds(bool compact, uint32_t lds) {
+    return with_bools([&](auto C) {
+        for (const void* k : {reinterpret_cast<const void*>(&wf_trav_tri_kernel<C(), false>), reinterpret_cast<const void*>(&wf_trav_tri_kernel<C(), true>)}) {
+            const hipError_t ek = hipFuncSetAttribute(k, hipFuncAttributeMaxDynamicSharedMemorySize, (int)lds);
+            if (ek != hipSuccess) return ek;
+        }
+        return hipSuccess;
+    }, compact);
+}
+
+}
```
